# inuyasha2012/vipsy

Hardware: AMD Instinct MI355X
Metric: ELBO-grad steps/sec, 1M persons x 500 items x 100-dim 2PL IRT (higher is better)
Workload: dtype f32

## Files before the change

vipsy_amd/csrc/k_mvn_fwd_b.hip:

```cpp

#define FB_THREADS 256
#define FB_WAVES 4

#define FB_WP 32
#define FB_A_BYTES 8192
#define FB_AUX_BYTES 1024
#define FB_IMG_BYTES (FB_A_BYTES + FB_AUX_BYTES)

__host__ __device__ inline int fb_tiles(int D) { return (pk_off_total(D) + 2 * pk_sec(D)) / 32; }
__host__ __device__ inline int64_t fb_img_floats(int D) {
    return (int64_t)fb_tiles(D) * (FB_IMG_BYTES / 4) + (pk_off_total(D) / 8 + 8 + 3) / 4 * 4;
}
__host__ __device__ inline size_t fb_wave_floats(int D, int J) {
    const size_t w = enc_p_wave_floats(D, J);
    return w < 2048 ? 2048 : w;
}
__host__ __device__ inline size_t fb_lds_bytes(int D, int J) {
    return FB_WAVES * fb_wave_floats(D, J) * sizeof(float) +
           (size_t)(pk_off_total(D) / 8 + 4) / 4 * 16 + 512;
}

#define FB_SC_BLOCKS 64
#define FB_SC_PART 16
#define FB_NSCALES (FB_SC_PART + 4 * FB_SC_BLOCKS)
#define FB_SC_BLOCKS 64
__device__ __forceinline__ void enc_scales_block_max(int blk, int D, int J, const float* __restrict__ W1, const float* __restrict__ b1,
                                                     const float* __restrict__ W21, const float* __restrict__ b21,
                                                     const float* __restrict__ W22, const float* __restrict__ b22,
                                                     float& mw, float& mb, float& m1, float& l1) {
    const int tid = threadIdx.x, lane = tid & 63, wave = tid >> 6;
    const int T = D * (D + 1) / 2;
    const int gt = blk * 256 + tid, gn = FB_SC_BLOCKS * 256;
    mw = 0.f; mb = 0.f; m1 = 0.f; l1 = 0.f;
    auto max4 = [&](const float* __restrict__ w, int n) __attribute__((always_inline)) {
        if (((uintptr_t)w & 15) == 0 && (n & 3) == 0) {
            const f32x4* w4 = (const f32x4*)w;
            const int n4 = n >> 2;
            for (int e = gt; e < n4; e += 4 * gn) {
                f32x4 v[4];
#pragma unroll
                for (int q = 0; q < 4; ++q) v[q] = (e + q * gn < n4) ? w4[e + q * gn] : f32x4{0.f, 0.f, 0.f, 0.f};
#pragma unroll
                for (int q = 0; q < 4; ++q)
                    mw = fmaxf(fmaxf(mw, fmaxf(fabsf(v[q][0]), fabsf(v[q][1]))), fmaxf(fabsf(v[q][2]), fabsf(v[q][3])));
            }
        } else {
            for (int e = gt; e < n; e += gn) mw = fmaxf(mw, fabsf(w[e]));
        }
    };
    max4(W21, D * 64);
    max4(W22, T * 64);
    for (int e = gt; e < D; e += gn) mb = fmaxf(mb, fabsf(b21[e]));
    for (int e = gt; e < T; e += gn) mb = fmaxf(mb, fabsf(b22[e]));
    for (int u = blk * 4 + wave; u < 64; u += FB_SC_BLOCKS * 4) {
        float sacc = 0.f;
        const float* wu = W1 + (int64_t)u * J;
        for (int j0 = 0; j0 < J; j0 += 512) {
            float w[8];
#pragma unroll
            for (int q = 0; q < 8; ++q) w[q] = (j0 + 64 * q + lane < J) ? fabsf(wu[j0 + 64 * q + lane]) : 0.f;
#pragma unroll
            for (int q = 0; q < 8; ++q)
                if (j0 + 64 * q + lane < J) { sacc += w[q]; m1 = fmaxf(m1, w[q]); }
        }
        sacc = wave_sum(sacc) + fabsf(b1[u]);
        l1 = fmaxf(l1, sacc);
    }
    mw = wave_max_dpp(mw); mb = wave_max_dpp(mb); m1 = wave_max_dpp(m1);
}
__global__ __launch_bounds__(256) void k_enc_scales_max(int D, int J, const float* __restrict__ W1, const float* __restrict__ b1,
                                                        const float* __restrict__ W21, const float* __restrict__ b21,
                                                        const float* __restrict__ W22, const float* __restrict__ b22,
                                                        float* __restrict__ sc) {
    float mw, mb, m1, l1;
    enc_scales_block_max(blockIdx.x, D, J, W1, b1, W21, b21, W22, b22, mw, mb, m1, l1);
    if ((threadIdx.x & 63) == 0) {
        uint32_t* w = (uint32_t*)(sc + 11);
        atomicMax(w + 0, __builtin_bit_cast(uint32_t, mw)); atomicMax(w + 1, __builtin_bit_cast(uint32_t, mb));
        atomicMax(w + 2, __builtin_bit_cast(uint32_t, m1)); atomicMax(w + 3, __builtin_bit_cast(uint32_t, l1));
    }
}
__device__ __forceinline__ void enc_scales_from_max(float mw, float mb, float m1, float l1, float* __restrict__ sc) {
    const float hbound = 1.001f * (fmaxf(l1, 0.f) + log1pf(expf(-fabsf(l1)))) + 1e-30f;
    const int sw1 = f16_scale_exp(m1), sh = f16_scale_exp(hbound);
    int sw = f16_scale_exp(mw), sb = f16_scale_exp(mb), eb = sw + sh - sb;
    if (eb > 15) { sw -= eb - 15; eb = 15; }
    if (eb < -14) { sb = sw + sh + 14; eb = -14; }
    sc[0] = ldexpf(1.f, sw1); sc[1] = ldexpf(1.f, -sw1);
    sc[2] = ldexpf(1.f, sw); sc[3] = ldexpf(1.f, sh); sc[4] = ldexpf(1.f, -(sw + sh));
    sc[5] = ldexpf(1.f, sb); sc[6] = ldexpf(1.f, eb);
    sc[7] = hbound; sc[8] = mw; sc[9] = mb; sc[10] = m1;
}
__global__ void k_enc_scales(float* __restrict__ sc) {
    if (threadIdx.x != 0 || blockIdx.x != 0) return;
    enc_scales_from_max(sc[11], sc[12], sc[13], sc[14], sc);
}

template <bool DIRECT = false>
__device__ __forceinline__ void pack_heads_b_tile(int T, int n_off_groups, const float* __restrict__ Wp, const float* __restrict__ bp,
                                                  const uint32_t* __restrict__ gtab, float w_scale, float b_scale,
                                                  uint8_t* __restrict__ img, uint32_t* __restrict__ gt2, int D = 0,
                                                  const float* __restrict__ W21 = nullptr, const float* __restrict__ b21 = nullptr,
                                                  const float* __restrict__ W22 = nullptr, const float* __restrict__ b22 = nullptr,
                                                  uint32_t* __restrict__ gtab_out = nullptr) {
    uint8_t* out = img + (int64_t)T * FB_IMG_BYTES;
    const int tid = threadIdx.x;
    const int Tt = D * (D + 1) / 2;
    if constexpr (DIRECT) {
        if (tid < 4) {
            const int G = 4 * T + tid;
            int src;
            uint32_t c, cn = 0u;
            pk_decode(8 * G, D, Tt, src, c);
            gtab_out[G] = c;
            if (G < n_off_groups) {
                if (G + 1 < n_off_groups) pk_decode(8 * (G + 1), D, Tt, src, cn);
                const uint32_t k = (c >> 12) & 0xFFFFu, l0 = c & 0xFFFu;
                const bool last = (G + 1 == n_off_groups) || (((cn >> 12) & 0xFFFFu) != k);
                gt2[G] = (4u * l0) | ((4u * k) << 12) | (last ? 0x80000000u : 0u);
            }
        }
    } else if (tid < 4 && 4 * T + tid < n_off_groups) {
        const int G = 4 * T + tid;
        const uint32_t c = gtab[G], k = (c >> 12) & 0xFFFFu, l0 = c & 0xFFFu;
        const bool last = (G + 1 == n_off_groups) || (((gtab[G + 1] >> 12) & 0xFFFFu) != k);
        gt2[G] = (4u * l0) | ((4u * k) << 12) | (last ? 0x80000000u : 0u);
    }
    const int row = (tid >> 3) & 31;
    const float* wrow;
    int bsrc = -1;
    if constexpr (DIRECT) {
        uint32_t gc;
        pk_decode(T * 32 + row, D, Tt, bsrc, gc);
        wrow = bsrc < 0 ? nullptr : (bsrc < Tt ? W22 + (int64_t)bsrc * 64 : W21 + (int64_t)(bsrc - Tt) * 64);
    } else {
        wrow = Wp + ((int64_t)T * 32 + row) * 64;
    }
    float v[8];
#pragma unroll
    for (int i = 0; i < 8; ++i) {
        const int e = tid + 256 * i;
        const int j = e & 7, lane = (e >> 3) & 63, sx = e >> 9;
        const int half = lane >> 5;
        v[i] = wrow ? wrow[16 * sx + 8 * (j >> 2) + 4 * half + (j & 3)] : 0.f;
    }
    float bv = 0.f;
    const bool bias_thread = tid < 256 && (tid & 7) < 2;
    if (bias_thread) {
        if constexpr (DIRECT) {
            bv = bsrc < 0 ? 0.f : (bsrc < Tt ? b22[bsrc] : b21[bsrc - Tt]);
        } else {
            bv = bp[T * 32 + (tid >> 3)];
        }
    }
#pragma unroll
    for (int i = 0; i < 8; ++i) {
        const int e = tid + 256 * i;
        const int j = e & 7, lane = (e >> 3) & 63, sx = e >> 9;
        uint16_t* o = (uint16_t*)(out + sx * 1024 + lane * 16) + j;
        split2h_bits(w_scale * v[i], o[0], o[2048]);
    }
    for (int e = tid; e < FB_AUX_BYTES / 2; e += 256) {
        const int j = e & 7;
        uint16_t w = 0;
        if (e < 256 && j < 2) {
            uint16_t bh, bl;
            split2h_bits(b_scale * bv, bh, bl);
            w = j == 0 ? bh : bl;
        }
        ((uint16_t*)(out + FB_A_BYTES))[e] = w;
    }
}
__global__ __launch_bounds__(256) void k_pack_heads_b(int n_tiles, int n_off_groups, const float* __restrict__ Wp, const float* __restrict__ bp,
                               const uint32_t* __restrict__ gtab, const float* __restrict__ sc, uint8_t* __restrict__ img,
                               uint32_t* __restrict__ gt2) {
    if ((int)blockIdx.x >= n_tiles) return;
    pack_heads_b_tile(blockIdx.x, n_off_groups, Wp, bp, gtab, sc[2], sc[5], img, gt2);
}

#define FB_W1_KS 4096
__host__ __device__ inline int64_t fb_w1img_floats(int J) { return (int64_t)((J + 15) / 16) * (FB_W1_KS / 4); }
__device__ __forceinline__ void pack_w1_b_kstep(int ks, int J, const float* __restrict__ W1, float w1_scale, uint8_t* __restrict__ w1img) {
    uint8_t* out = w1img + (int64_t)ks * FB_W1_KS;
    if (blockDim.x != 256) {
        for (int e = threadIdx.x; e < 2 * 64 * 8; e += blockDim.x) {
            const int j = e & 7, lane = (e >> 3) & 63, ht = e >> 9;
            const int half = lane >> 5, hh = 32 * ht + (lane & 31);
            const int it = 16 * ks + 8 * half + j;
            const float w = it < J ? w1_scale * W1[(int64_t)hh * J + it] : 0.f;
            uint16_t* o = (uint16_t*)(out + (ht * 2) * 1024 + lane * 16) + j;
            split2h_bits(w, o[0], o[512]);
        }
        return;
    }
    float v[4];
#pragma unroll
    for (int i = 0; i < 4; ++i) {
        const int e = threadIdx.x + 256 * i;
        const int j = e & 7, lane = (e >> 3) & 63, ht = e >> 9;
        const int half = lane >> 5, hh = 32 * ht + (lane & 31);
        const int it = 16 * ks + 8 * half + j;
        v[i] = it < J ? w1_scale * W1[(int64_t)hh * J + it] : 0.f;
    }
#pragma unroll
    for (int i = 0; i < 4; ++i) {
        const int e = threadIdx.x + 256 * i;
        const int j = e & 7, lane = (e >> 3) & 63, ht = e >> 9;
        uint16_t* o = (uint16_t*)(out + (ht * 2) * 1024 + lane * 16) + j;
        split2h_bits(v[i], o[0], o[512]);
    }
}
__global__ void k_pack_w1_b(int J, const float* __restrict__ W1, const float* __restrict__ sc, uint8_t* __restrict__ w1img) {
    pack_w1_b_kstep(blockIdx.x, J, W1, sc[0], w1img);
}

__device__ __forceinline__ f16x8 fb_y_frag(const uint32_t* yw) {
    typedef uint32_t u32x4y __attribute__((ext_vector_type(4)));
    const uint32_t w0 = yw[0], w1 = yw[1];
    u32x4y q;
#pragma unroll
    for (int d = 0; d < 4; ++d) {
        const uint32_t src = (d >> 1) ? w1 : w0;
        const uint32_t t = (d & 1) ? __builtin_amdgcn_perm(0u, src, 0x0c030c02u) : __builtin_amdgcn_perm(0u, src, 0x0c010c00u);
        q[d] = (t & 0x00010001u) * 0x3C00u | ((t & 0x00800080u) << 8);
    }
    return __builtin_bit_cast(f16x8, q);
}

__device__ __forceinline__ void fb_split8(const float* v, bf16x8& fh, bf16x8& fm, bf16x8& fl) {
    typedef uint32_t u32x4v __attribute__((ext_vector_type(4)));
    u32x4v ph, pm, pl;
#pragma unroll
    for (int q = 0; q < 4; ++q) {
        uint32_t hb[2], mb[2], lb[2];
#pragma unroll
        for (int e = 0; e < 2; ++e) {
            const float x = v[2 * q + e];
            hb[e] = __builtin_bit_cast(uint32_t, x) & 0xffff0000u;
            const float r1 = x - __builtin_bit_cast(float, hb[e]);
            mb[e] = __builtin_bit_cast(uint32_t, r1) & 0xffff0000u;
            const float r2 = r1 - __builtin_bit_cast(float, mb[e]);
            lb[e] = __builtin_bit_cast(uint32_t, r2) & 0xffff0000u;
        }
        ph[q] = hb[1] | (hb[0] >> 16);
        pm[q] = mb[1] | (mb[0] >> 16);
        pl[q] = lb[1] | (lb[0] >> 16);
    }
    fh = __builtin_bit_cast(bf16x8, ph);
    fm = __builtin_bit_cast(bf16x8, pm);
    fl = __builtin_bit_cast(bf16x8, pl);
}

#define FB_SPLIT_MAX 8192
template <bool SPLIT>
__global__ __launch_bounds__(FB_THREADS, 1) void k_mvn_enc_fwd_b(
    EncDims dm, const uint8_t* __restrict__ y, const int64_t* __restrict__ rows, int64_t gid0,
    const uint8_t* __restrict__ w1img, const float* __restrict__ b1, const uint8_t* __restrict__ img,
    const uint32_t* __restrict__ gt2, const float* __restrict__ sc , const float* __restrict__ eps_in, uint64_t seed,
    uint32_t step, const uint32_t* __restrict__ step_dev, uint32_t stream, float* __restrict__ h_out,
    float* __restrict__ x_out, float* __restrict__ eps_out, float* __restrict__ ldT, float* __restrict__ ent_out,
    float* __restrict__ hT_out , float* __restrict__ epsT_out ,
    uint8_t* __restrict__ ximg_out ,
    uint16_t* __restrict__ hs_out ,
    int64_t i_base = 0 ) {
    if (step_dev) step = *step_dev;
    extern __shared__ __attribute__((aligned(16))) float smem[];
    typedef uint32_t u32x4w __attribute__((ext_vector_type(4)));
    constexpr int H = 64;
    const int D = dm.D, J = dm.J;
    const int DS = pk_dse(D), DX = (D + 3) & ~3;
    const int YS = ef_ys(J);
    const int tid = threadIdx.x, lane = tid & 63, wave = __builtin_amdgcn_readfirstlane(tid >> 6);
    const int half = lane >> 5, l31 = lane & 31;
    float* R1 = smem + wave * fb_wave_floats(D, J);
    int8_t* Yi = (int8_t*)R1;
    float* S1 = SPLIT ? smem : R1;
    float* eps_lds = S1;
    float* x_lds = S1 + FB_WP * DS;
    uint32_t* gt_lds = (uint32_t*)(smem + FB_WAVES * fb_wave_floats(D, J));
    float* ent_s = (float*)(gt_lds + ((pk_off_total(D) / 8 + 4) / 4 * 4));
    const int64_t i0 = i_base + (SPLIT ? (int64_t)blockIdx.x * FB_WP : ((int64_t)blockIdx.x * FB_WAVES + wave) * FB_WP);
    const int p = l31;
    const int64_t i = i0 + p;
    const bool wave_live = i0 < dm.nb;
#ifdef FB_STAMPS
    uint64_t fst_[10]; int fsn_ = 0;
#define FSTAMP() do { __builtin_amdgcn_s_waitcnt(0); fst_[fsn_++] = __builtin_amdgcn_s_memtime(); } while (0)
#else
#define FSTAMP() do {} while (0)
#endif
    FSTAMP();

    const int n_off = pk_off_total(D) / 32;
    const int n_sec = pk_sec(D) / 32;
    const int t_end = n_off + 2 * n_sec;
    constexpr int FB_GQ = 5;
    uint32_t gtv[FB_GQ];
#pragma unroll
    for (int q = 0; q < FB_GQ; ++q) { const int e = tid + q * FB_THREADS; gtv[q] = e < 4 * n_off ? gt2[e] : 0u; }
    const float w1_inv = sc[1], h_scale = sc[3], acc_inv = sc[4];

    const int n_ydma = (32 * J + 1023) / 1024;
    const bool ydense = !rows && ((J >> 2) & 1) && i0 + FB_WP <= dm.nb && (i0 * J + (int64_t)n_ydma * 1024 <= dm.nb * (int64_t)J) &&
                        (size_t)n_ydma * 1024 <= fb_wave_floats(D, J) * sizeof(float);
    const int ysr = ydense ? J : YS;
    constexpr int FB_EQ = 16;
    f32x4 zq[FB_EQ];
    const int nblk = D >> 2;
    auto draw_eps = [&]() __attribute__((always_inline)) {
#pragma unroll
        for (int q = 0; q < FB_EQ; ++q) {
            const int e = lane + 64 * q;
            f32x4 z = {0.f, 0.f, 0.f, 0.f};
            if ((!SPLIT || (q & (FB_WAVES - 1)) == wave) && e < FB_WP * nblk) {
                const int pp = e / nblk, blk = e - pp * nblk;
                int64_t ii = i0 + pp;
                if (ii >= dm.nb) ii = dm.nb - 1;
                if (eps_in) {
                    z = *(const f32x4*)(eps_in + ii * D + 4 * blk);
                } else {
                    const int64_t row = rows ? rows[ii] : ii;
                    z = philox_normal4(seed, step, stream, gid0 + row, (uint32_t)blk);
                }
            }
            zq[q] = z;
        }
    };
    if (ydense) {
        const uint8_t* src = y + i0 * J + 16 * lane;
        const uint32_t lb = lds_addr_uniform(R1);
        for (int d = 0; d < n_ydma; ++d) dma16(src + d * 1024, lb + (uint32_t)d * 1024u);
        draw_eps();
        vx_wait_vmem();
    } else {
        constexpr int PB = 16, MAXLD = 4;
        const int YW = YS / 4, JW = J / 4;
        const int nld = (JW + 63) >> 6, nch = (YW + 63) >> 6;
        uint32_t* Yw = (uint32_t*)R1;
        int64_t rowb = 0;
        {
            const int64_t ii = i0 + l31;
            if (ii < dm.nb) rowb = (rows ? rows[ii] : ii) * J;
        }
        const int rowb_lo = (int)(uint32_t)rowb, rowb_hi = (int)(uint32_t)((uint64_t)rowb >> 32);
        if constexpr (SPLIT) {
            const int n_ks_all = (J + 15) / 16, ks_per = (n_ks_all + FB_WAVES - 1) / FB_WAVES;
            const int w_lo = 4 * ks_per * wave;
            const int wpp = 4 * ks_per;
            const int ppl = 64 / wpp > 0 ? 64 / wpp : 1;
            const int pl = lane / wpp, wl = lane - pl * wpp;
            draw_eps();
            for (int p0 = 0; p0 < FB_WP; p0 += ppl * 8) {
                uint32_t v[8];
#pragma unroll
                for (int u = 0; u < 8; ++u) {
                    const int pp = p0 + ppl * u + pl;
                    const int ppc = pp < FB_WP ? pp : FB_WP - 1;
                    const uint64_t rb = ((uint64_t)(uint32_t)__builtin_amdgcn_ds_bpermute(4 * ppc, rowb_hi) << 32) |
                                        (uint32_t)__builtin_amdgcn_ds_bpermute(4 * ppc, rowb_lo);
                    v[u] = 0u;
                    if (pl < ppl && pp < FB_WP && i0 + pp < dm.nb && w_lo + wl < JW) v[u] = ((const uint32_t*)(y + (int64_t)rb))[w_lo + wl];
                }
#pragma unroll
                for (int u = 0; u < 8; ++u) {
                    const int pp = p0 + ppl * u + pl;
                    if (pl < ppl && pp < FB_WP && w_lo + wl < YW) Yw[pp * YW + w_lo + wl] = v[u];
                }
            }
        } else
        for (int p0 = 0; p0 < FB_WP; p0 += PB) {
            uint32_t v[PB][MAXLD];
#pragma unroll
            for (int u = 0; u < PB; ++u) {
                const int pp = p0 + u;
                const uint64_t rb = ((uint64_t)(uint32_t)__builtin_amdgcn_readlane(rowb_hi, pp) << 32) |
                                    (uint32_t)__builtin_amdgcn_readlane(rowb_lo, pp);
                const uint32_t* src = (const uint32_t*)(y + (int64_t)rb) + lane;
                const bool live = i0 + pp < dm.nb;
#pragma unroll
                for (int c = 0; c < MAXLD; ++c) {
                    v[u][c] = 0u;
                    if (c < nld && live && lane + 64 * c < JW) v[u][c] = src[64 * c];
                }
            }
            if (p0 == 0) draw_eps();
#pragma unroll
            for (int u = 0; u < PB; ++u) {
                uint32_t* dst = Yw + (p0 + u) * YW + lane;
#pragma unroll
                for (int c = 0; c < MAXLD + 1; ++c)
                    if (c < nch && lane + 64 * c < YW) dst[64 * c] = c < MAXLD ? v[u][c < MAXLD ? c : 0] : 0u;
            }
        }
    }
#pragma unroll
    for (int q = 0; q < FB_GQ; ++q) { const int e = tid + q * FB_THREADS; if (e < 4 * n_off) gt_lds[e] = gtv[q]; }
    __builtin_amdgcn_wave_barrier();
    FSTAMP();
    f16x8 hb[2][4];
    {
        f32x16 hreg[2];
        f32x16 acc0 = zero16(), acc1 = zero16();
        const int n_ks = (J + 15) / 16;
        auto loadA = [&](f16x8 (&Af)[4], int ks) __attribute__((always_inline)) {
            ks = ks < n_ks ? ks : n_ks - 1;
            const uint8_t* src = w1img + (int64_t)ks * FB_W1_KS + lane * 16;
#pragma unroll
            for (int f = 0; f < 4; ++f) Af[f] = *(const f16x8*)(src + f * 1024);
        };
        auto compute = [&](const f16x8 (&Af)[4], int ks) __attribute__((always_inline)) {
            const f16x8 yb = fb_y_frag((const uint32_t*)(Yi + p * ysr + 16 * ks + 8 * half));
            acc0 = mfma_f16(Af[1], yb, acc0); acc1 = mfma_f16(Af[3], yb, acc1);
            acc0 = mfma_f16(Af[0], yb, acc0); acc1 = mfma_f16(Af[2], yb, acc1);
        };
        if constexpr (SPLIT) {
            const int ks_per = (n_ks + FB_WAVES - 1) / FB_WAVES;
            const int ks_lo = ks_per * wave, ks_hi = (ks_lo + ks_per < n_ks) ? ks_lo + ks_per : n_ks;
            f16x8 A[4][4];
            loadA(A[0], ks_lo); loadA(A[1], ks_lo + 1); loadA(A[2], ks_lo + 2);
            for (int c = ks_lo; c < ks_hi; c += 4) {
#pragma unroll
                for (int u = 0; u < 4; ++u) {
                    loadA(A[(u + 3) & 3], c + u + 3);
                    if (c + u < ks_hi) compute(A[u], c + u);
                }
            }
            __builtin_amdgcn_wave_barrier();
#pragma unroll
            for (int r = 0; r < 16; ++r) { R1[r * 64 + lane] = acc0[r]; R1[(16 + r) * 64 + lane] = acc1[r]; }
            __syncthreads();
            const size_t wstride = fb_wave_floats(D, J);
#pragma unroll
            for (int r = 0; r < 16; ++r) {
                float a0 = smem[r * 64 + lane], a1 = smem[(16 + r) * 64 + lane];
#pragma unroll
                for (int w = 1; w < FB_WAVES; ++w) { a0 += smem[w * wstride + r * 64 + lane]; a1 += smem[w * wstride + (16 + r) * 64 + lane]; }
                acc0[r] = a0; acc1[r] = a1;
            }
            __syncthreads();
        } else {
            f16x8 A[4][4];
            loadA(A[0], 0); loadA(A[1], 1); loadA(A[2], 2);
            for (int c = 0; c < n_ks; c += 4) {
#pragma unroll
                for (int u = 0; u < 4; ++u) {
                    loadA(A[(u + 3) & 3], c + u + 3);
                    if (c + u < n_ks) compute(A[u], c + u);
                }
            }
        }
#pragma unroll
        for (int ht = 0; ht < 2; ++ht) {
#pragma unroll
            for (int g = 0; g < 4; ++g) {
                const int hh0 = 32 * ht + 8 * g + 4 * half;
                const float4 bb = *(const float4*)(b1 + hh0);
                float4 hv;
                hv.x = softplusf_(fmaf((ht ? acc1 : acc0)[4 * g + 0], w1_inv, bb.x));
                hv.y = softplusf_(fmaf((ht ? acc1 : acc0)[4 * g + 1], w1_inv, bb.y));
                hv.z = softplusf_(fmaf((ht ? acc1 : acc0)[4 * g + 2], w1_inv, bb.z));
                hv.w = softplusf_(fmaf((ht ? acc1 : acc0)[4 * g + 3], w1_inv, bb.w));
                hreg[ht][4 * g + 0] = hv.x; hreg[ht][4 * g + 1] = hv.y;
                hreg[ht][4 * g + 2] = hv.z; hreg[ht][4 * g + 3] = hv.w;
                if ((SPLIT ? wave == ht : true) && i < dm.nb) *(float4*)(h_out + i * H + hh0) = hv;
            }
        }
        if (hT_out && i < dm.nb) {
#pragma unroll
            for (int ht = 0; ht < 2; ++ht)
                if (SPLIT ? wave == 2 + ht : true)
#pragma unroll
                    for (int r = 0; r < 16; ++r) hT_out[(int64_t)(32 * ht + crow32(r, half)) * dm.nb + i] = hreg[ht][r];
        }
        if (hs_out && i < dm.nb) {
            const int64_t plane = (int64_t)64 * dm.nb;
#pragma unroll
            for (int ht = 0; ht < 2; ++ht)
                if (SPLIT ? wave == ht : true)
#pragma unroll
                    for (int r = 0; r < 16; ++r) {
                        const int64_t o = (int64_t)(32 * ht + crow32(r, half)) * dm.nb + i;
                        split2h_bits(hreg[ht][r] * h_scale, hs_out[o], hs_out[plane + o]);
                    }
        }
#pragma unroll
        for (int s = 0; s < 4; ++s) {
            float v[8];
#pragma unroll
            for (int j = 0; j < 8; ++j) v[j] = hreg[s >> 1][8 * (s & 1) + j];
            split2h_frag(v, h_scale, hb[0][s], hb[1][s]);
        }
    }
    __builtin_amdgcn_wave_barrier();
    FSTAMP();
    if constexpr (SPLIT) {
        __syncthreads();
        for (int e = tid; e < FB_WP * DX / 4; e += FB_THREADS) *(f32x4*)(x_lds + 4 * e) = f32x4{0.f, 0.f, 0.f, 0.f};
        for (int e = tid; e < FB_WP * (DS - D) / 4; e += FB_THREADS) {
            const int pp = e / ((DS - D) / 4), c = e - pp * ((DS - D) / 4);
            *(f32x4*)(eps_lds + pp * DS + D + 4 * c) = f32x4{0.f, 0.f, 0.f, 0.f};
        }
#pragma unroll
        for (int q = 0; q < FB_EQ; ++q) {
            const int e = lane + 64 * q;
            if ((q & (FB_WAVES - 1)) == wave && e < FB_WP * nblk) {
                const int pp = e / nblk, blk = e - pp * nblk;
                *(f32x4*)(eps_lds + pp * DS + 4 * blk) = zq[q];
                if (i0 + pp < dm.nb) *(f32x4*)(eps_out + (i0 + pp) * D + 4 * blk) = zq[q];
            }
        }
    } else {
        for (int e = lane; e < FB_WP * (DS + DX) / 4; e += 64) *(f32x4*)(S1 + 4 * e) = f32x4{0.f, 0.f, 0.f, 0.f};
        __builtin_amdgcn_wave_barrier();
#pragma unroll
        for (int q = 0; q < FB_EQ; ++q) {
            const int e = lane + 64 * q;
            if (e < FB_WP * nblk) {
                const int pp = e / nblk, blk = e - pp * nblk;
                *(f32x4*)(eps_lds + pp * DS + 4 * blk) = zq[q];
                if (i0 + pp < dm.nb) *(f32x4*)(eps_out + (i0 + pp) * D + 4 * blk) = zq[q];
            }
        }
        __builtin_amdgcn_wave_barrier();
        if (epsT_out && i < dm.nb) {
#pragma unroll 4
            for (int k = half; k < D; k += 2) epsT_out[(int64_t)k * dm.nb + i] = eps_lds[p * DS + k];
        }
    }
    float ent_acc = 0.f;
    const float* ep = eps_lds + p * DS;
    float* xp = x_lds + p * DX;
    struct TileRegs { f16x8 a[2][4]; f16x8 bias; };
    auto pull = [&](TileRegs& R, int t) __attribute__((always_inline)) {
        const int tc = t < t_end ? t : t_end - 1;
        const uint8_t* gb = img + (int64_t)tc * FB_IMG_BYTES + lane * 16;
        R.bias = *(const f16x8*)(gb + FB_A_BYTES);
#pragma unroll
        for (int sp = 1; sp >= 0; --sp)
#pragma unroll
            for (int s = 0; s < 4; ++s) R.a[sp][s] = *(const f16x8*)(gb + (sp * 4 + s) * 1024);
    };
    f16x8 cfrag;
    {
        const _Float16 c16 = (_Float16)sc[6];
#pragma unroll
        for (int j = 0; j < 8; ++j) cfrag[j] = c16;
    }
    auto mma_all = [&](const TileRegs& R) __attribute__((always_inline)) -> f32x16 {
        f32x16 a = mfma_f16(R.bias, cfrag, zero16());
#pragma unroll
        for (int s = 0; s < 4; ++s) a = mfma_f16(R.a[1][s], hb[0][s], a);
#pragma unroll
        for (int s = 0; s < 4; ++s) a = mfma_f16(R.a[0][s], hb[1][s], a);
#pragma unroll
        for (int s = 0; s < 4; ++s) a = mfma_f16(R.a[0][s], hb[0][s], a);
        return a;
    };
    float cur_part = 0.f;
    const char* ep_h = (const char*)(ep + 4 * half);
    char* xp_b = (char*)xp;
    struct EpiOps { float4 e4[4]; };
    auto epi_read = [&](EpiOps& E, const uint4& c) __attribute__((always_inline)) {
        E.e4[0] = *(const float4*)(ep_h + (c.x & 0xFFFu));
        E.e4[1] = *(const float4*)(ep_h + (c.y & 0xFFFu));
        E.e4[2] = *(const float4*)(ep_h + (c.z & 0xFFFu));
        E.e4[3] = *(const float4*)(ep_h + (c.w & 0xFFFu));
    };
    auto epi_group = [&](const f32x16& a, const float4& e, uint32_t code, int g) __attribute__((always_inline)) {
        cur_part = fmaf(a[4 * g + 0], e.x, cur_part);
        cur_part = fmaf(a[4 * g + 1], e.y, cur_part);
        cur_part = fmaf(a[4 * g + 2], e.z, cur_part);
        cur_part = fmaf(a[4 * g + 3], e.w, cur_part);
        if (__builtin_expect((int)code < 0, 0)) {
            const float tot = half_sum32(cur_part) * acc_inv;
            if (half == 0) {
                if (SPLIT) atomicAdd((float*)(xp_b + ((code >> 12) & 0xFFFu)), tot);
                else *(float*)(xp_b + ((code >> 12) & 0xFFFu)) = tot;
            }
            cur_part = 0.f;
        }
    };

    FSTAMP();
    __syncthreads();
    FSTAMP();
    if constexpr (SPLIT) {
        if (epsT_out && i < dm.nb) {
#pragma unroll 4
            for (int k = 2 * wave + half; k < D; k += 2 * FB_WAVES) epsT_out[(int64_t)k * dm.nb + i] = eps_lds[p * DS + k];
        }
    }
    int t_lo = 0, t_hi = n_off;
    if (SPLIT) {
        const int nr = (n_off / 2 < FB_WAVES) ? n_off / 2 : FB_WAVES;
        const int qn = (n_off / nr) & ~1;
        t_lo = wave < nr ? wave * qn : n_off;
        t_hi = (wave >= nr - 1) ? n_off : t_lo + qn;
    }
    TileRegs RA, RB;
    pull(RA, t_lo);
    f32x16 accP = zero16();
    uint4 codeP = make_uint4(0, 0, 0, 0);

    auto off_iter = [&](TileRegs& Rc, TileRegs& Rn, int t, auto firstc) __attribute__((always_inline)) {
        constexpr bool first = decltype(firstc)::value;
        EpiOps E;
        if constexpr (!first) epi_read(E, codeP);
        pull(Rn, t + 1);
        f32x16 a = mfma_f16(Rc.bias, cfrag, zero16());
        a = mfma_f16(Rc.a[1][0], hb[0][0], a);
        a = mfma_f16(Rc.a[1][1], hb[0][1], a);
        if constexpr (!first) epi_group(accP, E.e4[0], codeP.x, 0);
        a = mfma_f16(Rc.a[1][2], hb[0][2], a);
        a = mfma_f16(Rc.a[1][3], hb[0][3], a);
        a = mfma_f16(Rc.a[0][0], hb[1][0], a);
        if constexpr (!first) epi_group(accP, E.e4[1], codeP.y, 1);
        a = mfma_f16(Rc.a[0][1], hb[1][1], a);
        a = mfma_f16(Rc.a[0][2], hb[1][2], a);
        a = mfma_f16(Rc.a[0][3], hb[1][3], a);
        if constexpr (!first) epi_group(accP, E.e4[2], codeP.z, 2);
        a = mfma_f16(Rc.a[0][0], hb[0][0], a);
        a = mfma_f16(Rc.a[0][1], hb[0][1], a);
        if constexpr (!first) epi_group(accP, E.e4[3], codeP.w, 3);
        a = mfma_f16(Rc.a[0][2], hb[0][2], a);
        a = mfma_f16(Rc.a[0][3], hb[0][3], a);
        accP = a;
        const uint4 cv = *(const uint4*)(gt_lds + 4 * t);
        codeP.x = __builtin_amdgcn_readfirstlane(cv.x); codeP.y = __builtin_amdgcn_readfirstlane(cv.y);
        codeP.z = __builtin_amdgcn_readfirstlane(cv.z); codeP.w = __builtin_amdgcn_readfirstlane(cv.w);
    };
    if (!SPLIT || t_lo < t_hi) {
        off_iter(RA, RB, t_lo, std::true_type{});
        off_iter(RB, RA, t_lo + 1, std::false_type{});
        for (int t = t_lo + 2; t < t_hi; t += 2) {
            off_iter(RA, RB, t, std::false_type{});
            off_iter(RB, RA, t + 1, std::false_type{});
        }
        {
            EpiOps E;
            epi_read(E, codeP);
            epi_group(accP, E.e4[0], codeP.x, 0);
            epi_group(accP, E.e4[1], codeP.y, 1);
            epi_group(accP, E.e4[2], codeP.z, 2);
            epi_group(accP, E.e4[3], codeP.w, 3);
        }
        if (SPLIT) {
            const float tot = half_sum32(cur_part) * acc_inv;
            if (half == 0) atomicAdd((float*)(xp_b + ((codeP.w >> 12) & 0xFFFu)), tot);
            cur_part = 0.f;
        }
    }
    FSTAMP();
    if (SPLIT) __syncthreads();
    FSTAMP();
    auto tile_sec = [&](const f32x16& a, int t2) __attribute__((always_inline)) {
        const bool is_diag = t2 < n_off + n_sec;
        const int k0 = 32 * (t2 - (is_diag ? n_off : n_off + n_sec));
#pragma unroll
        for (int g = 0; g < 4; ++g) {
            const int kk = k0 + 8 * g + 4 * half;
            if (kk < D) {
                f32x4 xo = *(const f32x4*)(xp + kk);
                if (is_diag) {
                    const f32x4 ev = *(const f32x4*)(ep + kk);
#pragma unroll
                    for (int j = 0; j < 4; ++j) {
                        const float mkk = a[4 * g + j] * acc_inv;
                        const float ld = __expf(mkk);
                        xo[j] = fmaf(ld, ev[j], xo[j]);
                        ent_acc += mkk;
                        if (i < dm.nb) ldT[(int64_t)(kk + j) * dm.nb + i] = ld;
                    }
                } else {
#pragma unroll
                    for (int j = 0; j < 4; ++j) xo[j] = fmaf(a[4 * g + j], acc_inv, xo[j]);
                }
                *(f32x4*)(xp + kk) = xo;
            }
        }
    };
    auto sec_iter = [&](TileRegs& Rc, TileRegs& Rn, int t) __attribute__((always_inline)) {
        if (t + 1 < t_end) pull(Rn, t + 1);
        const f32x16 a = mma_all(Rc);
        tile_sec(a, t);
    };
    if (SPLIT) {
        for (int ts = wave; ts < n_sec; ts += FB_WAVES) {
            pull(RA, n_off + ts);
            tile_sec(mma_all(RA), n_off + ts);
            pull(RA, n_off + n_sec + ts);
            tile_sec(mma_all(RA), n_off + n_sec + ts);
        }
        const float ea = ent_acc + __shfl_xor(ent_acc, 32, 64);
        if (half == 0) ent_s[wave * FB_WP + p] = ea;
        __syncthreads();
        ent_acc = (ent_s[p] + ent_s[FB_WP + p]) + (ent_s[2 * FB_WP + p] + ent_s[3 * FB_WP + p]);
    } else {
        for (int t = n_off; t < t_end; t += 2) {
            sec_iter(RA, RB, t);
            sec_iter(RB, RA, t + 1);
        }
    }
    vx_wait_vmem();
    __builtin_amdgcn_wave_barrier();
    FSTAMP();
    const int e_lo = SPLIT ? tid : lane, e_st = SPLIT ? FB_THREADS : 64;
    if (ximg_out && i0 < (dm.nb + 63) / 64 * 64) {
        const int pvi = (int)((dm.nb - i0) < FB_WP ? (dm.nb - i0) : FB_WP);
        uint8_t* out = ximg_out + (i0 >> 6) * LH_XT_BYTES;
        const int pbase = (int)(i0 & 63);
        for (int e = e_lo; e < FB_WP * 2 * LB_NKS; e += e_st) {
            int pp, ch;
            if (e < 4 * 3 * 32) {
                const int blk = e >> 5, r = e & 31;
                pp = 8 * (blk / 3) + (r >> 2);
                ch = 4 * (blk % 3) + (r & 3);
            } else {
                const int r = e - 4 * 3 * 32;
                pp = 8 * (r >> 4) + ((r >> 1) & 7);
                ch = 12 + (r & 1);
            }
            float v[8];
#pragma unroll
            for (int j = 0; j < 8; ++j) {
                const int k = 8 * ch + j;
                v[j] = (pp < pvi) ? (k < D ? x_lds[pp * DX + k] : (k == D ? 1.0f : 0.f)) : 0.f;
            }
            f16x8 fh, fl;
            if (lh_split_x(v, fh, fl)) atomicOr((uint32_t*)(ximg_out + (dm.nb + 63) / 64 * (int64_t)LH_XT_BYTES), 1u);
            const uint32_t o = lb_xoff(pbase + pp, ch);
            *(f16x8*)(out + o) = fh;
            *(f16x8*)(out + LB_PLANE + o) = fl;
        }
    }
    if (wave_live) {
        const int pv = (int)((dm.nb - i0) < FB_WP ? (dm.nb - i0) : FB_WP);
        const int c4 = D >> 2;
        for (int e = e_lo; e < pv * c4; e += e_st) {
            const int pp = e / c4, c = e - pp * c4;
            *(f32x4*)(x_out + (i0 + pp) * D + 4 * c) = *(const f32x4*)(x_lds + pp * DX + 4 * c);
        }
        if (!SPLIT) ent_acc += __shfl_xor(ent_acc, 32, 64);
        if ((SPLIT ? wave == FB_WAVES - 1 : true) && half == 0 && i < dm.nb) {
            float s = 0.f;
            for (int k = 0; k < D; k += 4) {
                const f32x4 e = *(const f32x4*)(eps_lds + p * DS + k);
                s += e[0] * e[0]; s += e[1] * e[1]; s += e[2] * e[2]; s += e[3] * e[3];
            }
            ent_out[i] = 0.5f * s + ent_acc;
        }
    }
#ifdef FB_STAMPS
    FSTAMP();
    if (blockIdx.x == 1 && lane == 0)
        printf("FSTAMPS blk %d wave %d: y+draw %llu fc1 %llu eps %llu bar %llu off %llu bar %llu sec %llu out %llu total %llu\n", (int)blockIdx.x, wave,
               fst_[1] - fst_[0], fst_[2] - fst_[1], fst_[3] - fst_[2], fst_[4] - fst_[3], fst_[5] - fst_[4], fst_[6] - fst_[5], fst_[7] - fst_[6],
               fst_[8] - fst_[7], fst_[8] - fst_[0]);
#endif
}


#define NB_THREADS 256
#define NB_WAVES 4
__host__ __device__ inline size_t nb_lds_bytes(int J) {
    return (size_t)NB_WAVES * norm_fast_wave_floats(J) * sizeof(float) + 2 * 6 * 1024;
}

__global__ __launch_bounds__(NB_THREADS, 2) void k_norm_enc_fwd_b(
    EncDims dm, const uint8_t* __restrict__ y, const int64_t* __restrict__ rows, const float* __restrict__ W1,
    const float* __restrict__ b1, const float* __restrict__ W21, const float* __restrict__ b21,
    const float* __restrict__ W22, const float* __restrict__ b22, float* __restrict__ h_out,
    float* __restrict__ loc_out, float* __restrict__ raw_out) {
    extern __shared__ __attribute__((aligned(16))) float smem[];
    typedef uint32_t u32x4w __attribute__((ext_vector_type(4)));
    typedef uint32_t u32x2w __attribute__((ext_vector_type(2)));
    constexpr int H = 64;
    const int J = dm.J, YS = ef_ys(J);
    const int tid = threadIdx.x, lane = tid & 63, wave = tid >> 6, half = lane >> 5, l31 = lane & 31;
    float* R1 = smem + wave * norm_fast_wave_floats(J);
    const int8_t* Yi = (const int8_t*)R1;
    char* frag = (char*)(smem + NB_WAVES * norm_fast_wave_floats(J));
    const int64_t i0 = ((int64_t)blockIdx.x * NB_WAVES + wave) * EP_WP;
    const int p = l31;
    const int64_t i = i0 + p;
    const int n_ydma = (32 * J + 1023) / 1024;
    const bool ydense = !rows && ((J >> 2) & 1) && i0 + EP_WP <= dm.nb && (i0 * J + (int64_t)n_ydma * 1024 <= dm.nb * (int64_t)J);
    const int ysr = ydense ? J : YS;
    if (ydense) {
        const uint8_t* src = y + i0 * J + 16 * lane;
        const uint32_t lb = lds_addr_uniform(R1);
        for (int d = 0; d < n_ydma; ++d) dma16(src + d * 1024, lb + (uint32_t)d * 1024u);
    } else {
        const int YW = YS / 4, JW = J / 4;
        uint32_t* Yw = (uint32_t*)R1;
        const int64_t ip = i0 + l31;
        const int64_t myrow = ip < dm.nb ? (rows ? rows[ip] : ip) : (int64_t)-1;
        const int row_lo = (int)(uint32_t)myrow, row_hi = (int)(uint32_t)((uint64_t)myrow >> 32);
        if (YW >= 64) {
#pragma unroll 4
            for (int pp = 0; pp < EP_WP; ++pp) {
                const int64_t row = (int64_t)(((uint64_t)(uint32_t)__builtin_amdgcn_readlane(row_hi, pp) << 32) |
                                              (uint32_t)__builtin_amdgcn_readlane(row_lo, pp));
                for (int wq = lane; wq < YW; wq += 64) {
                    uint32_t v = 0u;
                    if (wq < JW && row >= 0) v = *(const uint32_t*)(y + row * J + 4 * wq);
                    Yw[pp * YW + wq] = v;
                }
            }
        } else {
#pragma unroll 4
            for (int e = lane; e < EP_WP * YW; e += 64) {
                const int pp = e / YW, wq = e - pp * YW;
                const int64_t row = (int64_t)(((uint64_t)(uint32_t)__shfl(row_hi, pp, 64) << 32) | (uint32_t)__shfl(row_lo, pp, 64));
                uint32_t v = 0u;
                if (wq < JW && row >= 0) v = *(const uint32_t*)(y + row * J + 4 * wq);
                Yw[e] = v;
            }
        }
    }
    const int n_ks = (J + 15) / 16;
    const int hh = tid >> 2, q = tid & 3;
    const float* wrow = W1 + (int64_t)hh * J + 4 * q;
    auto fetch_w = [&](int ks) -> float4 {
        const int j0 = 16 * ks + 4 * q;
        return (ks < n_ks && j0 + 4 <= J) ? *(const float4*)(wrow + 16 * ks) : make_float4(0.f, 0.f, 0.f, 0.f);
    };
    char* wdst = frag + ((hh >> 5) * 3) * 1024 + (32 * (q >> 1) + (hh & 31)) * 16 + 8 * (q & 1);
    auto put_w = [&](const float4& w, int buf) {
        const float v[4] = {w.x, w.y, w.z, w.w};
        uint16_t t[3][4];
#pragma unroll
        for (int e = 0; e < 4; ++e) {
            const __bf16 a = (__bf16)v[e];
            const float r1 = v[e] - (float)a;
            const __bf16 m = (__bf16)r1;
            const __bf16 l = (__bf16)(r1 - (float)m);
            t[0][e] = __builtin_bit_cast(uint16_t, a); t[1][e] = __builtin_bit_cast(uint16_t, m); t[2][e] = __builtin_bit_cast(uint16_t, l);
        }
#pragma unroll
        for (int sp = 0; sp < 3; ++sp) {
            const u32x2w pk = {(uint32_t)t[sp][0] | ((uint32_t)t[sp][1] << 16), (uint32_t)t[sp][2] | ((uint32_t)t[sp][3] << 16)};
            *(u32x2w*)(wdst + buf * 6144 + sp * 1024) = pk;
        }
    };
    put_w(fetch_w(0), 0);
    constexpr int NB_PF = 4;
    float4 wq[NB_PF];
#pragma unroll
    for (int u = 0; u < NB_PF; ++u) wq[u] = fetch_w(1 + u);
    vx_wait_vmem();
    __syncthreads();
    f32x16 acc0 = zero16(), acc1 = zero16();
    for (int ks0 = 0; ks0 < n_ks; ks0 += NB_PF) {
#pragma unroll
      for (int u = 0; u < NB_PF; ++u) {
        const int ks = ks0 + u;
        if (ks >= n_ks) break;
        const int buf = ks & 1;
        const float4 wcur = wq[u];
        wq[u] = fetch_w(ks + 1 + NB_PF);
        const char* fb = frag + buf * 6144 + lane * 16;
        bf16x8 A[6];
#pragma unroll
        for (int f = 0; f < 6; ++f) A[f] = *(const bf16x8*)(fb + f * 1024);
        const uint32_t* yw = (const uint32_t*)(Yi + p * ysr + 16 * ks + 8 * half);
        const u32x2w w = {yw[0], yw[1]};
        u32x4w qv;
#pragma unroll
        for (int d = 0; d < 4; ++d) {
            const uint32_t src = w[d >> 1];
            const uint32_t t = (d & 1) ? __builtin_amdgcn_perm(0u, src, 0x0c030c02u) : __builtin_amdgcn_perm(0u, src, 0x0c010c00u);
            qv[d] = (t & 0x00010001u) * 0x3F80u | ((t & 0x00800080u) << 8);
        }
        const bf16x8 yb = __builtin_bit_cast(bf16x8, qv);
        acc0 = mfma_bf16(A[2], yb, acc0); acc1 = mfma_bf16(A[5], yb, acc1);
        acc0 = mfma_bf16(A[1], yb, acc0); acc1 = mfma_bf16(A[4], yb, acc1);
        acc0 = mfma_bf16(A[0], yb, acc0); acc1 = mfma_bf16(A[3], yb, acc1);
        if (ks + 1 < n_ks) put_w(wcur, buf ^ 1);
        __syncthreads();
      }
    }
    if (i0 >= dm.nb) return;
    float sl = 0.f, sr = 0.f;
#pragma unroll
    for (int ht = 0; ht < 2; ++ht)
#pragma unroll
        for (int g = 0; g < 4; ++g) {
            const int hh0 = 32 * ht + 8 * g + 4 * half;
            const float4 bb = *(const float4*)(b1 + hh0);
            const float4 w21 = make_float4(W21[hh0], W21[hh0 + 1], W21[hh0 + 2], W21[hh0 + 3]);
            const float4 w22 = make_float4(W22[hh0], W22[hh0 + 1], W22[hh0 + 2], W22[hh0 + 3]);
            float4 hv;
            hv.x = softplusf_((ht ? acc1 : acc0)[4 * g + 0] + bb.x);
            hv.y = softplusf_((ht ? acc1 : acc0)[4 * g + 1] + bb.y);
            hv.z = softplusf_((ht ? acc1 : acc0)[4 * g + 2] + bb.z);
            hv.w = softplusf_((ht ? acc1 : acc0)[4 * g + 3] + bb.w);
            sl += hv.x * w21.x + hv.y * w21.y + hv.z * w21.z + hv.w * w21.w;
            sr += hv.x * w22.x + hv.y * w22.y + hv.z * w22.z + hv.w * w22.w;
            if (i < dm.nb) *(float4*)(h_out + i * H + hh0) = hv;
        }
    sl = half_sum32(sl);
    sr = half_sum32(sr);
    if (half == 0 && i < dm.nb) {
        loc_out[i] = sl + b21[0];
        raw_out[i] = sr + b22[0];
    }
}


#define NH_MAX_BLOCKS 64
__host__ __device__ inline int64_t nh_pack_floats(int J) { return fb_w1img_floats(J) + 16 + NH_MAX_BLOCKS; }

__global__ __launch_bounds__(256) void k_norm_pack_max(int J, const float* __restrict__ W1, float* __restrict__ part) {
    __shared__ float red[4];
    float m = 0.f;
    const int n4 = 64 * J / 4;
    const f32x4* w4 = (const f32x4*)W1;
    for (int e = blockIdx.x * 256 + threadIdx.x; e < n4; e += NH_MAX_BLOCKS * 256) {
        const f32x4 v = w4[e];
        m = fmaxf(fmaxf(m, fmaxf(fabsf(v[0]), fabsf(v[1]))), fmaxf(fabsf(v[2]), fabsf(v[3])));
    }
    m = wave_max_dpp(m);
    if ((threadIdx.x & 63) == 0) red[threadIdx.x >> 6] = m;
    __syncthreads();
    if (threadIdx.x == 0) part[blockIdx.x] = fmaxf(fmaxf(red[0], red[1]), fmaxf(red[2], red[3]));
}
__global__ __launch_bounds__(256) void k_norm_pack_w1(int J, const float* __restrict__ W1, const float* __restrict__ part,
                                                      float* __restrict__ sc, uint8_t* __restrict__ w1img) {
    __shared__ float scl;
    if (threadIdx.x < 64) {
        const float m = wave_max_dpp(part[threadIdx.x]);
        if (threadIdx.x == 0) scl = ldexpf(1.f, f16_scale_exp(m));
    }
    __syncthreads();
    if (blockIdx.x == 0 && threadIdx.x == 0) { sc[0] = scl; sc[1] = 1.0f / scl; }
    pack_w1_b_kstep(blockIdx.x, J, W1, scl, w1img);
}

template <int NP>
__host__ __device__ inline size_t nh_wave_floats(int J) {
    const size_t a = (size_t)(32 * NP) * ef_ys(J) / 4, b = (size_t)(((32 * NP * J + 1023) / 1024) * 256);
    return ((a > b ? a : b) + 3) & ~(size_t)3;
}
template <int NP>
__host__ __device__ inline size_t nh_lds_bytes(int J) { return (4 / NP) * nh_wave_floats<NP>(J) * sizeof(float); }

template <int NP, int PF>
__global__ __launch_bounds__(64 * (4 / NP)) void k_norm_enc_fwd_h(
    EncDims dm, const uint8_t* __restrict__ y, const int64_t* __restrict__ rows, const uint8_t* __restrict__ w1img,
    const float* __restrict__ sc, const float* __restrict__ b1, const float* __restrict__ W21, const float* __restrict__ b21,
    const float* __restrict__ W22, const float* __restrict__ b22, float* __restrict__ h_out,
    float* __restrict__ loc_out, float* __restrict__ raw_out) {
    extern __shared__ __attribute__((aligned(16))) float smem[];
    constexpr int H = 64, WP = 32 * NP, NW = 4 / NP, RING = PF + 1;
    const int J = dm.J, YS = ef_ys(J);
    const int tid = threadIdx.x, lane = tid & 63, wave = tid >> 6, half = lane >> 5, l31 = lane & 31;
    float* R1 = smem + wave * nh_wave_floats<NP>(J);
    const int8_t* Yi = (const int8_t*)R1;
    const int64_t i0 = ((int64_t)blockIdx.x * NW + wave) * WP;
    if (i0 >= dm.nb) return;
#ifdef NH_STAMPS
    unsigned long long nst_[5]; int nsn_ = 0;
#define NSTAMP() do { __builtin_amdgcn_s_waitcnt(0); nst_[nsn_++] = __builtin_amdgcn_s_memtime(); } while (0)
#else
#define NSTAMP() do {} while (0)
#endif
    NSTAMP();
    const int n_ydma = (WP * J + 1023) / 1024;
    const bool ydense = !rows && ((J >> 2) & 1) && i0 + WP <= dm.nb && (i0 * J + (int64_t)n_ydma * 1024 <= dm.nb * (int64_t)J);
    const int ysr = ydense ? J : YS;
    const int n_ks = (J + 15) / 16;
    auto loadA = [&](f16x8 (&Af)[4], int ks) __attribute__((always_inline)) {
        ks = ks < n_ks ? ks : n_ks - 1;
        const uint8_t* src = w1img + (int64_t)ks * FB_W1_KS + lane * 16;
#pragma unroll
        for (int f = 0; f < 4; ++f) Af[f] = *(const f16x8*)(src + f * 1024);
    };
    f16x8 A[RING][4];
    if (ydense) {
        const uint8_t* src = y + i0 * J + 16 * lane;
        const uint32_t lb = lds_addr_uniform(R1);
        for (int d = 0; d < n_ydma; ++d) dma16(src + d * 1024, lb + (uint32_t)d * 1024u);
#pragma unroll
        for (int u = 0; u < PF; ++u) loadA(A[u], u);
        vx_wait_vmem();
    } else {
        const int YW = YS / 4, JW = J / 4;
        uint32_t* Yw = (uint32_t*)R1;
        for (int e = lane; e < WP * YW; e += 64) {
            const int pp = e / YW, wq = e - pp * YW;
            const int64_t ii = i0 + pp;
            uint32_t v = 0u;
            if (wq < JW && ii < dm.nb) {
                const int64_t row = rows ? rows[ii] : ii;
// ... 77 lines not shown
```

vipsy_amd/csrc/k_mvn_fwd_b2.hip:

```cpp

#define FB2_THREADS 256
#define FB2_WAVES 4
#define FB2_WP_OF(NS) (32 * (NS))

__host__ __device__ inline size_t fb2_wave_floats(int D, int J, int NS = 2) {
    const size_t a = (size_t)FB2_WP_OF(NS) * ef_ys(J) / 4, b = (size_t)FB2_WP_OF(NS) * pk_dse(D);
    return ((a > b ? a : b) + 3) & ~(size_t)3;
}
__host__ __device__ inline size_t fb2_lds_bytes(int D, int J, int NS = 2) {
    return FB2_WAVES * fb2_wave_floats(D, J, NS) * sizeof(float) + (size_t)(pk_off_total(D) / 8 + 4) / 4 * 16;
}

#define FB2_RING_SLOTS 3
__host__ __device__ inline size_t fb2_tbl_bytes(int D) { return (size_t)(pk_off_total(D) / 8 + 4) / 4 * 16; }
__host__ __device__ inline size_t fb2s_wave_floats(int D) {
    size_t f = (size_t)32 * D + 8;
    if (f < 3072) f = 3072;
    return (f + 3) & ~(size_t)3;
}
__host__ __device__ inline size_t fb2s_lds_bytes(int D) {
    return FB2_WAVES * fb2s_wave_floats(D) * sizeof(float) + fb2_tbl_bytes(D) + (size_t)FB2_RING_SLOTS * FB_IMG_BYTES;
}
__host__ __device__ inline bool fb2s_shape_ok(int D, int J) {
    return D % 4 == 0 && ((D >> 2) & 1) && D >= 80 && J % 4 == 0 && J <= 512 && J > 384 && pk_off_total(D) / 32 >= 4 &&
           2 * ((fb2s_lds_bytes(D) + 1279) / 1280 * 1280) <= 160 * 1024;
}
template <int NS, bool SH = false>
__global__ __launch_bounds__(FB2_THREADS, (NS == 1 ? 2 : 1)) void k_mvn_enc_fwd_b2(
    EncDims dm, const uint8_t* __restrict__ y, const int64_t* __restrict__ rows, int64_t gid0,
    const uint8_t* __restrict__ w1img, const float* __restrict__ b1, const uint8_t* __restrict__ img,
    const uint32_t* __restrict__ gt2, const float* __restrict__ sc , const float* __restrict__ eps_in,
    uint64_t seed, uint32_t step, const uint32_t* __restrict__ step_dev, uint32_t stream, float* __restrict__ h_out, float* __restrict__ x_out, float* __restrict__ eps_out, float* __restrict__ ldT,
    float* __restrict__ ent_out, float* __restrict__ hT_out, float* __restrict__ epsT_out, uint8_t* __restrict__ ximg_out,
    uint16_t* __restrict__ hs_out) {
    if (step_dev) step = *step_dev;
    extern __shared__ __attribute__((aligned(16))) float smem[];
    typedef uint32_t u32x4w __attribute__((ext_vector_type(4)));
    typedef uint32_t u32x2w __attribute__((ext_vector_type(2)));
    constexpr int H = 64, FB2_WP = FB2_WP_OF(NS);
    const int D = dm.D, J = dm.J;
    static_assert(!SH || NS == 1, "shared ring: one person set a wave");
    const int DS = SH ? D : pk_dse(D);
    const int YS = ef_ys(J);
    const int tid = threadIdx.x, lane = tid & 63, wave = __builtin_amdgcn_readfirstlane(tid >> 6);
    const int half = lane >> 5, l31 = lane & 31;
    const size_t WF = SH ? fb2s_wave_floats(D) : fb2_wave_floats(D, J, NS);
    float* R1 = smem + wave * WF;
    int8_t* Yi = (int8_t*)R1;
    float* eps_lds = R1;
    uint32_t* gt_lds = (uint32_t*)(smem + FB2_WAVES * WF);
    uint8_t* ring = (uint8_t*)gt_lds + fb2_tbl_bytes(D);
    const int64_t i0 = ((int64_t)blockIdx.x * FB2_WAVES + wave) * FB2_WP;
    const int p = l31;
    int64_t iu[NS];
#pragma unroll
    for (int u = 0; u < NS; ++u) iu[u] = i0 + 32 * u + p;

#ifdef FB2_STAMPS
    uint64_t st_[10]; int sn_ = 0;
    uint64_t w_lds_ = 0, w_vm_ = 0, w_bar_ = 0;
#define STAMP() do { __builtin_amdgcn_s_waitcnt(0); st_[sn_++] = __builtin_amdgcn_s_memtime(); } while (0)
#else
#define STAMP() do {} while (0)
#endif
    STAMP();
    const int n_off = pk_off_total(D) / 32;
    const int n_sec = pk_sec(D) / 32;
    const int t_end = n_off + 2 * n_sec;
    for (int e = tid; e < 4 * n_off; e += FB2_THREADS) gt_lds[e] = gt2[e];
    const float w1_inv = sc[1], h_scale = sc[3], acc_inv = sc[4];
    const uint32_t ring_lb = SH ? lds_addr_uniform(ring) : 0u;
    auto ring_dma = [&](int t, int slot) __attribute__((always_inline)) {
        const int tc = t < t_end ? t : t_end - 1;
        const uint8_t* gb = img + (int64_t)tc * FB_IMG_BYTES + lane * 16;
        const uint32_t lb = ring_lb + (uint32_t)slot * FB_IMG_BYTES;
        dma16(gb + wave * 1024, lb + (uint32_t)wave * 1024u);
        dma16(gb + (wave + 4) * 1024, lb + (uint32_t)(wave + 4) * 1024u);
        if (wave == 0) dma16(gb + 8 * 1024, lb + 8u * 1024u);
    };
    if constexpr (SH) { ring_dma(0, 0); ring_dma(1, 1); ring_dma(2, 2); }

    const bool qdma = SH && !rows && i0 + FB2_WP <= dm.nb && (i0 + FB2_WP - 1) * (int64_t)J + 512 <= dm.nb * (int64_t)J;
    auto stage_q = [&](int q, int slot) __attribute__((always_inline)) {
        if (qdma) {
            const uint32_t lb = lds_addr_uniform(R1) + (uint32_t)slot * 4096u;
#pragma unroll
            for (int d = 0; d < 4; ++d) {
                const int row = 8 * d + (lane >> 3), pos = lane & 7, c = pos ^ ((row ^ (row >> 3)) & 7);
                dma16(y + (i0 + row) * J + 128 * q + 16 * c, lb + (uint32_t)d * 1024u);
            }
        } else {
            uint32_t* Yw = (uint32_t*)R1 + slot * 1024;
            for (int e = lane; e < 32 * 32; e += 64) {
                const int row = e >> 5, w = e & 31, byte = 128 * q + 4 * w;
                const int64_t ii = i0 + row;
                uint32_t v = 0u;
                if (byte < J && ii < dm.nb) {
                    const int64_t rr = rows ? rows[ii] : ii;
                    v = *(const uint32_t*)(y + rr * J + byte);
                }
                Yw[row * 32 + 4 * ((w >> 2) ^ ((row ^ (row >> 3)) & 7)) + (w & 3)] = v;
            }
        }
    };
    const int n_ydma = (FB2_WP * J + 1023) / 1024;
    const bool ydense = !rows && ((J >> 2) & 1) && i0 + FB2_WP <= dm.nb && (i0 * J + (int64_t)n_ydma * 1024 <= dm.nb * (int64_t)J) &&
                        (size_t)n_ydma * 1024 <= fb2_wave_floats(D, J, NS) * sizeof(float);
    const int ysr = ydense ? J : YS;
    if constexpr (SH) {
        stage_q(0, 0); stage_q(1, 1); stage_q(2, 2);
        if (qdma) vx_wait_vmem();
    } else if (ydense) {
        const uint8_t* src = y + i0 * J + 16 * lane;
        const uint32_t lb = lds_addr_uniform(R1);
        for (int d = 0; d < n_ydma; ++d) dma16(src + d * 1024, lb + (uint32_t)d * 1024u);
        vx_wait_vmem();
    } else {
        const int YW = YS / 4, JW = J / 4;
        uint32_t* Yw = (uint32_t*)R1;
        for (int e = lane; e < FB2_WP * YW; e += 64) {
            const int pp = e / YW, wq = e - pp * YW;
            const int64_t ii = i0 + pp;
            uint32_t v = 0u;
            if (wq < JW && ii < dm.nb) {
                const int64_t row = rows ? rows[ii] : ii;
                v = *(const uint32_t*)(y + row * J + 4 * wq);
            }
            Yw[e] = v;
        }
    }
    __builtin_amdgcn_wave_barrier();
    STAMP();
    f16x8 hb[NS][2][4];
    {
        f32x16 acc[NS][2];
#pragma unroll
        for (int u = 0; u < NS; ++u) { acc[u][0] = zero16(); acc[u][1] = zero16(); }
        const int n_ks = (J + 15) / 16;
        auto loadA = [&](f16x8 (&Af)[4], int ks) __attribute__((always_inline)) {
            ks = ks < n_ks ? ks : n_ks - 1;
            const uint8_t* src = w1img + (int64_t)ks * FB_W1_KS + lane * 16;
#pragma unroll
            for (int f = 0; f < 4; ++f) Af[f] = *(const f16x8*)(src + f * 1024);
        };
        auto compute = [&](const f16x8 (&Af)[4], int ks) __attribute__((always_inline)) {
#pragma unroll
            for (int u = 0; u < NS; ++u) {
                const int8_t* yp = SH ? Yi + ((ks >> 3) == 3 ? 0 : (ks >> 3)) * 4096 + p * 128 + 16 * ((ks & 7) ^ ((p ^ (p >> 3)) & 7)) + 8 * half
                                      : Yi + (32 * u + p) * ysr + 16 * ks + 8 * half;
                const f16x8 yb = fb_y_frag((const uint32_t*)yp);
                acc[u][0] = mfma_f16(Af[1], yb, acc[u][0]); acc[u][1] = mfma_f16(Af[3], yb, acc[u][1]);
                acc[u][0] = mfma_f16(Af[0], yb, acc[u][0]); acc[u][1] = mfma_f16(Af[2], yb, acc[u][1]);
            }
        };
        {
            constexpr int RG = 8;
            f16x8 A[RG][4];
#pragma unroll
            for (int u = 0; u < RG - 1; ++u) loadA(A[u], u);
            for (int c = 0; c < n_ks; c += RG) {
                if constexpr (SH) {
                    if (c == 8) {
                        asm volatile("s_waitcnt lgkmcnt(0)" ::: "memory");
                        __builtin_amdgcn_wave_barrier();
                        stage_q(3, 0);
                    }
                    if (c == 24) {
                        if (qdma) vx_wait_vmem();
                        __builtin_amdgcn_wave_barrier();
                    }
                }
#pragma unroll
                for (int u = 0; u < RG; ++u) {
                    loadA(A[(u + RG - 1) % RG], c + u + RG - 1);
                    if (c + u < n_ks) compute(A[u], c + u);
                }
            }
        }
        STAMP();
        constexpr int ST_T = 36, ST_S = 40;
        constexpr bool SEQ = NS == 1;
        const bool coal = i0 + FB2_WP <= dm.nb && (dm.nb & 7) == 0 && hT_out && hs_out &&
                          (((uintptr_t)hT_out | (uintptr_t)hs_out) & 15) == 0 &&
                          WF * sizeof(float) >= (SEQ ? 128 * ST_S * 2 : 64 * ST_T * 4 + 128 * ST_S * 2);
        float* stT = R1;
        uint16_t* stS = SEQ ? (uint16_t*)R1 : (uint16_t*)(R1 + 64 * ST_T);
#pragma unroll
        for (int u = 0; u < NS; ++u) {
            const int64_t i = iu[u];
            f32x16 hreg[2];
#pragma unroll
            for (int ht = 0; ht < 2; ++ht) {
#pragma unroll
                for (int g = 0; g < 4; ++g) {
                    const int hh0 = 32 * ht + 8 * g + 4 * half;
                    const float4 bb = *(const float4*)(b1 + hh0);
                    float4 hv;
                    hv.x = softplusf_(fmaf(acc[u][ht][4 * g + 0], w1_inv, bb.x));
                    hv.y = softplusf_(fmaf(acc[u][ht][4 * g + 1], w1_inv, bb.y));
                    hv.z = softplusf_(fmaf(acc[u][ht][4 * g + 2], w1_inv, bb.z));
                    hv.w = softplusf_(fmaf(acc[u][ht][4 * g + 3], w1_inv, bb.w));
                    hreg[ht][4 * g + 0] = hv.x; hreg[ht][4 * g + 1] = hv.y;
                    hreg[ht][4 * g + 2] = hv.z; hreg[ht][4 * g + 3] = hv.w;
                    if (i < dm.nb) *(float4*)(h_out + i * H + hh0) = hv;
                }
            }
#pragma unroll
            for (int s = 0; s < 4; ++s) {
                float v[8];
#pragma unroll
                for (int j = 0; j < 8; ++j) v[j] = hreg[s >> 1][8 * (s & 1) + j];
                split2h_frag(v, h_scale, hb[u][0][s], hb[u][1][s]);
            }
            if (coal) {
                __builtin_amdgcn_wave_barrier();
#pragma unroll
                for (int ht = 0; ht < 2; ++ht)
#pragma unroll
                    for (int r = 0; r < 16; ++r) stT[(32 * ht + crow32(r, half)) * ST_T + p] = hreg[ht][r];
                const int64_t c0 = i0 + 32 * u;
                if constexpr (SEQ) {
                    __builtin_amdgcn_wave_barrier();
#ifndef FB2_NO_HT
#pragma unroll
                    for (int it = 0; it < 8; ++it) {
                        const int e = lane + 64 * it, hh = e >> 3, g = e & 7;
                        *(f32x4*)(hT_out + (int64_t)hh * dm.nb + c0 + 4 * g) = *(const f32x4*)(stT + hh * ST_T + 4 * g);
                    }
#endif
                    __builtin_amdgcn_wave_barrier();
                }
#pragma unroll
                for (int t2 = 0; t2 < 2; ++t2)
#pragma unroll
                    for (int s = 0; s < 4; ++s) {
                        const u32x4w w = __builtin_bit_cast(u32x4w, hb[u][t2][s]);
#pragma unroll
                        for (int j = 0; j < 8; ++j) {
                            const int hh = 32 * (s >> 1) + crow32(8 * (s & 1) + j, half);
                            stS[(64 * t2 + hh) * ST_S + p] = (uint16_t)((j & 1) ? (w[j >> 1] >> 16) : (w[j >> 1] & 0xFFFFu));
                        }
                    }
                __builtin_amdgcn_wave_barrier();
                if constexpr (!SEQ) {
#pragma unroll
                    for (int it = 0; it < 8; ++it) {
                        const int e = lane + 64 * it, hh = e >> 3, g = e & 7;
                        *(f32x4*)(hT_out + (int64_t)hh * dm.nb + c0 + 4 * g) = *(const f32x4*)(stT + hh * ST_T + 4 * g);
                    }
                }
#pragma unroll
                for (int it = 0; it < 8; ++it) {
                    const int e = lane + 64 * it, row = e >> 2, g = e & 3;
                    *(u32x4w*)(hs_out + (int64_t)row * dm.nb + c0 + 8 * g) = *(const u32x4w*)(stS + row * ST_S + 8 * g);
                }
            } else if (hT_out && i < dm.nb) {
#pragma unroll
                for (int ht = 0; ht < 2; ++ht)
#pragma unroll
                    for (int r = 0; r < 16; ++r) hT_out[(int64_t)(32 * ht + crow32(r, half)) * dm.nb + i] = hreg[ht][r];
            }
            if (!coal && hs_out && i < dm.nb) {
                const int64_t plane = (int64_t)64 * dm.nb;
#pragma unroll
                for (int ht = 0; ht < 2; ++ht)
#pragma unroll
                    for (int r = 0; r < 16; ++r) {
                        const int64_t o = (int64_t)(32 * ht + crow32(r, half)) * dm.nb + i;
                        split2h_bits(hreg[ht][r] * h_scale, hs_out[o], hs_out[plane + o]);
                    }
            }
        }
    }
    STAMP();
    __builtin_amdgcn_wave_barrier();
    const int nblk = D >> 2;
    for (int e = lane; e < FB2_WP * DS / 4 + (SH ? 2 : 0); e += 64) *(f32x4*)(R1 + 4 * e) = f32x4{0.f, 0.f, 0.f, 0.f};
    __builtin_amdgcn_wave_barrier();
#pragma unroll 5
    for (int e = lane; e < FB2_WP * nblk; e += 64) {
        const int pp = e / nblk, blk = e - pp * nblk;
        int64_t ii = i0 + pp;
        const bool live = ii < dm.nb;
        if (!live) ii = dm.nb - 1;
        f32x4 z;
        if (eps_in) {
            z = *(const f32x4*)(eps_in + ii * D + 4 * blk);
        } else {
            const int64_t row = rows ? rows[ii] : ii;
            z = philox_normal4(seed, step, stream, gid0 + row, (uint32_t)blk);
        }
        *(f32x4*)(eps_lds + pp * DS + 4 * blk) = z;
    }
    __builtin_amdgcn_wave_barrier();
    const bool coalE = i0 + FB2_WP <= dm.nb && (dm.nb & 3) == 0 && epsT_out && ((uintptr_t)epsT_out & 15) == 0;
    if (coalE) {
        constexpr int PG = FB2_WP / 4;
        for (int e = lane; e < D * PG; e += 64) {
            const int k = e / PG, g = e - k * PG;
            const float* ec = eps_lds + 4 * g * DS + k;
            *(f32x4*)(epsT_out + (int64_t)k * dm.nb + i0 + 4 * g) = f32x4{ec[0], ec[DS], ec[2 * DS], ec[3 * DS]};
        }
    }
    float eps2[NS];
#pragma unroll
    for (int u = 0; u < NS; ++u) {
        const float* er = eps_lds + (32 * u + p) * DS;
        if (!coalE && epsT_out && iu[u] < dm.nb) {
#pragma unroll 4
            for (int k = half; k < D; k += 2) epsT_out[(int64_t)k * dm.nb + iu[u]] = er[k];
        }
        float s2 = 0.f;
        for (int k = 0; k < D; ++k) s2 = fmaf(er[k], er[k], s2);
        eps2[u] = s2;
    }
    STAMP();
    struct TileRegs { f16x8 a[2][4]; f16x8 bias; };
    auto pull = [&](TileRegs& R, int t) __attribute__((always_inline)) {
        const int tc = t < t_end ? t : t_end - 1;
        const uint8_t* gb = img + (int64_t)tc * FB_IMG_BYTES + lane * 16;
        R.bias = *(const f16x8*)(gb + FB_A_BYTES);
#pragma unroll
        for (int sp = 1; sp >= 0; --sp)
#pragma unroll
            for (int s = 0; s < 4; ++s) R.a[sp][s] = *(const f16x8*)(gb + (sp * 4 + s) * 1024);
    };
    f16x8 cfrag;
    {
        const _Float16 c16 = (_Float16)sc[6];
#pragma unroll
        for (int j = 0; j < 8; ++j) cfrag[j] = c16;
    }
    auto mma_all = [&](const TileRegs& R, int u) __attribute__((always_inline)) -> f32x16 {
        f32x16 a = mfma_f16(R.bias, cfrag, zero16());
#pragma unroll
        for (int s = 0; s < 4; ++s) a = mfma_f16(R.a[1][s], hb[u][0][s], a);
#pragma unroll
        for (int s = 0; s < 4; ++s) a = mfma_f16(R.a[0][s], hb[u][1][s], a);
#pragma unroll
        for (int s = 0; s < 4; ++s) a = mfma_f16(R.a[0][s], hb[u][0][s], a);
        return a;
    };
    float cur_part[NS];
    const char* ep_h[NS];
    float* xrow[NS];
    float* xst[NS];
    const bool whole = i0 + FB2_WP <= dm.nb;
    const int st_sh = whole ? (NS == 2 ? 6 : 5) : 0;
#pragma unroll
    for (int u = 0; u < NS; ++u) {
        cur_part[u] = 0.f;
        ep_h[u] = (const char*)(eps_lds + (32 * u + p) * DS + 4 * half);
        xrow[u] = x_out + (iu[u] < dm.nb ? iu[u] : dm.nb - 1) * D;
        xst[u] = whole ? eps_out + i0 * D + 32 * u + p : xrow[u];
    }
    struct EpiOps { float4 e4[NS][4]; };
    auto epi_read = [&](EpiOps& E, const uint4& c) __attribute__((always_inline)) {
#pragma unroll
        for (int u = 0; u < NS; ++u) {
            E.e4[u][0] = *(const float4*)(ep_h[u] + (c.x & 0xFFFu));
            E.e4[u][1] = *(const float4*)(ep_h[u] + (c.y & 0xFFFu));
            E.e4[u][2] = *(const float4*)(ep_h[u] + (c.z & 0xFFFu));
            E.e4[u][3] = *(const float4*)(ep_h[u] + (c.w & 0xFFFu));
        }
    };
    auto epi_group = [&](const f32x16 (&a)[NS], const EpiOps& E, uint32_t code, int g) __attribute__((always_inline)) {
#pragma unroll
        for (int j = 0; j < 4; ++j)
#pragma unroll
            for (int u = 0; u < NS; ++u) {
                const float ev = j == 0 ? E.e4[u][g].x : j == 1 ? E.e4[u][g].y : j == 2 ? E.e4[u][g].z : E.e4[u][g].w;
                float av = a[u][4 * g + j];
                if (g == 0 && j == 0) av = __builtin_bit_cast(float, __builtin_amdgcn_mov_dpp(__builtin_bit_cast(int, av), 0xE4, 0xF, 0xF, true));
                asm volatile("v_fmac_f32 %0, %1, %2" : "+v"(cur_part[u]) : "v"(av), "v"(ev));
            }
        if (__builtin_expect((int)code < 0, 0)) {
#pragma unroll
            for (int u = 0; u < NS; ++u) {
                const float tot = half_sum32(cur_part[u]) * acc_inv;
                if (half == 0 && iu[u] < dm.nb) *(float*)((char*)xst[u] + (((code >> 12) & 0xFFFu) << st_sh)) = tot;
                cur_part[u] = 0.f;
            }
        }
    };

    if constexpr (SH) vx_wait_vmem();
    __syncthreads();
    TileRegs RA, RB;
    int s_rd = 1;
    auto ring_read = [&](TileRegs& R, int slot) __attribute__((always_inline)) {
        const uint8_t* lb = ring + slot * FB_IMG_BYTES + lane * 16;
        R.bias = *(const f16x8*)(lb + FB_A_BYTES);
#pragma unroll
        for (int sp = 1; sp >= 0; --sp)
#pragma unroll
            for (int s = 0; s < 4; ++s) R.a[sp][s] = *(const f16x8*)(lb + (sp * 4 + s) * 1024);
    };
    f32x16 accP[NS];
#pragma unroll
    for (int u = 0; u < NS; ++u) accP[u] = zero16();
    uint4 codeP = make_uint4(0, 0, 0, 0);
    auto off_iter = [&](TileRegs& Rc, TileRegs& Rn, int t, auto firstc) __attribute__((always_inline)) {
        constexpr bool first = decltype(firstc)::value;
        EpiOps E;
        if constexpr (!first) epi_read(E, codeP);
        if constexpr (SH) ring_read(Rn, s_rd); else pull(Rn, t + 1);
        f32x16 a[NS];
#pragma unroll
        for (int u = 0; u < NS; ++u) a[u] = mfma_f16(Rc.bias, cfrag, zero16());
#pragma unroll
        for (int s = 0; s < 2; ++s)
#pragma unroll
            for (int u = 0; u < NS; ++u) a[u] = mfma_f16(Rc.a[1][s], hb[u][0][s], a[u]);
        if constexpr (!first) epi_group(accP, E, codeP.x, 0);
#pragma unroll
        for (int s = 2; s < 4; ++s)
#pragma unroll
            for (int u = 0; u < NS; ++u) a[u] = mfma_f16(Rc.a[1][s], hb[u][0][s], a[u]);
#pragma unroll
        for (int u = 0; u < NS; ++u) a[u] = mfma_f16(Rc.a[0][0], hb[u][1][0], a[u]);
        if constexpr (!first) epi_group(accP, E, codeP.y, 1);
#pragma unroll
        for (int s = 1; s < 4; ++s)
#pragma unroll
            for (int u = 0; u < NS; ++u) a[u] = mfma_f16(Rc.a[0][s], hb[u][1][s], a[u]);
        if constexpr (!first) epi_group(accP, E, codeP.z, 2);
#pragma unroll
        for (int s = 0; s < 2; ++s)
#pragma unroll
            for (int u = 0; u < NS; ++u) a[u] = mfma_f16(Rc.a[0][s], hb[u][0][s], a[u]);
        if constexpr (!first) epi_group(accP, E, codeP.w, 3);
#pragma unroll
        for (int s = 2; s < 4; ++s)
#pragma unroll
            for (int u = 0; u < NS; ++u) a[u] = mfma_f16(Rc.a[0][s], hb[u][0][s], a[u]);
#pragma unroll
        for (int u = 0; u < NS; ++u) accP[u] = a[u];
        const uint4 cv = *(const uint4*)(gt_lds + 4 * t);
        codeP.x = __builtin_amdgcn_readfirstlane(cv.x); codeP.y = __builtin_amdgcn_readfirstlane(cv.y);
        codeP.z = __builtin_amdgcn_readfirstlane(cv.z); codeP.w = __builtin_amdgcn_readfirstlane(cv.w);
        if constexpr (SH) {
#ifdef FB2_STAMPS
            const uint64_t tw0_ = __builtin_amdgcn_s_memtime();
#endif
            asm volatile("s_waitcnt lgkmcnt(0)" ::: "memory");
#ifdef FB2_STAMPS
            const uint64_t tw1_ = __builtin_amdgcn_s_memtime();
#endif
            if (wave == 0) __builtin_amdgcn_s_waitcnt(0x0F70 | 3); else __builtin_amdgcn_s_waitcnt(0x0F70 | 2);
#ifdef FB2_STAMPS
            const uint64_t tw2_ = __builtin_amdgcn_s_memtime();
#endif
            __builtin_amdgcn_s_barrier();
#ifdef FB2_STAMPS
            { const uint64_t tw3_ = __builtin_amdgcn_s_memtime(); w_lds_ += tw1_ - tw0_; w_vm_ += tw2_ - tw1_; w_bar_ += tw3_ - tw2_; }
#endif
            ring_dma(t + 4, s_rd);
            s_rd = s_rd == FB2_RING_SLOTS - 1 ? 0 : s_rd + 1;
        }
    };
    if constexpr (SH) {
        ring_read(RA, 0);
        asm volatile("s_waitcnt lgkmcnt(0)" ::: "memory");
        __builtin_amdgcn_s_barrier();
        ring_dma(3, 0);
    } else {
        pull(RA, 0);
    }
    off_iter(RA, RB, 0, std::true_type{});
    off_iter(RB, RA, 1, std::false_type{});
    for (int t = 2; t < n_off; t += 2) {
        off_iter(RA, RB, t, std::false_type{});
        off_iter(RB, RA, t + 1, std::false_type{});
    }
    {
        EpiOps E;
        epi_read(E, codeP);
        epi_group(accP, E, codeP.x, 0);
        epi_group(accP, E, codeP.y, 1);
        epi_group(accP, E, codeP.z, 2);
        epi_group(accP, E, codeP.w, 3);
    }
    vx_wait_vmem();
    STAMP();
    float ent_acc[NS];
#pragma unroll
    for (int u = 0; u < NS; ++u) ent_acc[u] = 0.f;
    pull(RA, n_off);
    pull(RB, n_off + n_sec);
    for (int kb = 0; kb < n_sec; ++kb) {
        const int k0 = 32 * kb;
        if (k0 >= D) break;
        f32x4 xo[NS][4];
#pragma unroll
        for (int u = 0; u < NS; ++u) {
#pragma unroll
            for (int g = 0; g < 4; ++g) {
                const int kk = k0 + 8 * g + 4 * half;
#pragma unroll
                for (int j = 0; j < 4; ++j) xo[u][g][j] = (kk < D) ? xst[u][(int64_t)(kk + j) << st_sh] : 0.f;
            }
            if (k0 == 0 && half == 0) xo[u][0][0] = 0.f;
        }
        f32x16 aD[NS], aL[NS];
#pragma unroll
        for (int u = 0; u < NS; ++u) aD[u] = mma_all(RA, u);
        pull(RA, n_off + kb + 1);
#pragma unroll
        for (int u = 0; u < NS; ++u) aL[u] = mma_all(RB, u);
        pull(RB, n_off + n_sec + kb + 1);
#pragma unroll
        for (int u = 0; u < NS; ++u) {
            const bool live = iu[u] < dm.nb;
            const float* er = eps_lds + (32 * u + p) * DS;
#pragma unroll
            for (int g = 0; g < 4; ++g) {
                const int kk = k0 + 8 * g + 4 * half;
                if (kk < D) {
                    const f32x4 ev = *(const f32x4*)(er + kk);
                    f32x4 xn;
#pragma unroll
                    for (int j = 0; j < 4; ++j) {
                        const float mkk = aD[u][4 * g + j] * acc_inv;
                        const float ld = __expf(mkk);
                        xn[j] = fmaf(aL[u][4 * g + j], acc_inv, fmaf(ld, ev[j], xo[u][g][j]));
                        ent_acc[u] += mkk;
                        if (live) ldT[(int64_t)(kk + j) * dm.nb + iu[u]] = ld;
                    }
                    if (live) *(f32x4*)(xrow[u] + kk) = xn;
                }
            }
        }
    }
    vx_wait_vmem();
    for (int e = lane; e < FB2_WP * nblk; e += 64) {
        const int pp = e / nblk, blk = e - pp * nblk;
        if (i0 + pp < dm.nb) *(f32x4*)(eps_out + (i0 + pp) * D + 4 * blk) = *(const f32x4*)(eps_lds + pp * DS + 4 * blk);
    }
#pragma unroll
    for (int u = 0; u < NS; ++u) {
        ent_acc[u] += __shfl_xor(ent_acc[u], 32, 64);
        if (half == 0 && iu[u] < dm.nb) ent_out[iu[u]] = 0.5f * eps2[u] + ent_acc[u];
    }
    STAMP();
    if (ximg_out && i0 < (dm.nb + 63) / 64 * 64) {
        const int pbase = (int)(i0 & 63);
        vx_wait_vmem();
        __builtin_amdgcn_wave_barrier();
        const int pvi = (int)((dm.nb - i0) < FB2_WP ? (dm.nb - i0) : FB2_WP);
        uint8_t* out = ximg_out + (i0 >> 6) * LH_XT_BYTES;
        constexpr int XU = 7;
        static_assert((FB2_WP * 2 * LB_NKS) % (64 * XU) == 0, "x image work items");
        for (int e0 = lane; e0 < FB2_WP * 2 * LB_NKS; e0 += 64 * XU) {
            f32x4 q[XU][2];
            uint32_t off[XU];
#pragma unroll
            for (int w = 0; w < XU; ++w) {
                const int e = e0 + 64 * w;
                const int hs2 = e / (32 * 2 * LB_NKS), e2 = e - hs2 * (32 * 2 * LB_NKS);
                int pp, ch;
                if (e2 < 4 * 3 * 32) {
                    const int blk = e2 >> 5, r = e2 & 31;
                    pp = 8 * (blk / 3) + (r >> 2);
                    ch = 4 * (blk % 3) + (r & 3);
                } else {
                    const int r = e2 - 4 * 3 * 32;
                    pp = 8 * (r >> 4) + ((r >> 1) & 7);
                    ch = 12 + (r & 1);
                }
                pp += 32 * hs2;
                off[w] = lb_xoff(pbase + pp, ch);
                const float* xr = x_out + (i0 + (pp < pvi ? pp : 0)) * D;
#pragma unroll
                for (int h2 = 0; h2 < 2; ++h2) {
                    const int k0 = 8 * ch + 4 * h2;
                    f32x4 v = {0.f, 0.f, 0.f, 0.f};
                    if (pp < pvi) {
                        if (k0 < D) v = *(const f32x4*)(xr + k0);
                        else if (k0 == D) v[0] = 1.0f;
                    }
                    q[w][h2] = v;
                }
            }
#pragma unroll
            for (int w = 0; w < XU; ++w) {
                float v[8];
#pragma unroll
                for (int j = 0; j < 8; ++j) v[j] = q[w][j >> 2][j & 3];
                f16x8 fh, fl;
                if (lh_split_x(v, fh, fl)) atomicOr((uint32_t*)(ximg_out + (dm.nb + 63) / 64 * (int64_t)LH_XT_BYTES), 1u);
                *(f16x8*)(out + off[w]) = fh;
                *(f16x8*)(out + LB_PLANE + off[w]) = fl;
            }
        }
    }
#ifdef FB2_STAMPS
    STAMP();
    if ((blockIdx.x == 100 || blockIdx.x == 2000 || blockIdx.x == 5000) && lane == 0 && (wave == 0 || wave == 3))
        printf("STAMPS blk %d wave %d: y %llu fc1 %llu hout %llu eps %llu off %llu sec %llu ximg %llu total %llu | turn waits: lds %llu dma %llu barrier %llu\n",
               (int)blockIdx.x, wave, st_[1] - st_[0], st_[2] - st_[1], st_[3] - st_[2], st_[4] - st_[3], st_[5] - st_[4], st_[6] - st_[5],
               st_[7] - st_[6], st_[7] - st_[0], w_lds_, w_vm_, w_bar_);
#endif
}
```

vipsy_amd/csrc/k_mvn_score_b.hip:

```cpp
#pragma once

#define SB_THREADS 256
#define SB_WAVES 4
#define SB_WP 32

__host__ __device__ inline int sb_col_jb0(int c) { return c & ~3; }
__host__ __device__ inline int sb_col_tiles(int D, int c) { return (D - sb_col_jb0(c) + 31) / 32; }
__host__ __device__ inline int sb_tiles(int D) {
    int n = 0;
    for (int c = 0; c < D; ++c) n += sb_col_tiles(D, c);
    return n;
}
__host__ __device__ inline int sb_ds(int D) {
    int ds = (D + 32 + 3) & ~3;
    if (((ds >> 2) & 1) == 0) ds += 4;
    return ds;
}
__host__ __device__ inline size_t sb_lds_bytes(int D) { return (size_t)SB_WAVES * SB_WP * sb_ds(D) * sizeof(float); }
#define SBR_CONSUMERS 8
#define SBR_THREADS (64 * (SBR_CONSUMERS + 1))
__host__ __device__ inline size_t sbr_lds_bytes(int D) {
    return (size_t)SBR_CONSUMERS * SB_WP * sb_ds(D) * sizeof(float) + 2 * (size_t)FB_IMG_BYTES;
}
__host__ __device__ inline int64_t sb_img_floats(int D) { return (int64_t)sb_tiles(D) * (FB_IMG_BYTES / 4); }

__global__ __launch_bounds__(256) void k_pack_heads_col(int D, const float* __restrict__ W22, const float* __restrict__ b22,
                                                       const float* __restrict__ sc, uint8_t* __restrict__ img) {
    int t = blockIdx.x, c = D - 1;
    while (c > 0 && t >= sb_col_tiles(D, c)) { t -= sb_col_tiles(D, c); --c; }
    const int jb = sb_col_jb0(c) + 32 * t;
    const float w_scale = sc[2], b_scale = sc[5];
    uint8_t* out = img + (int64_t)blockIdx.x * FB_IMG_BYTES;
    const int tid = threadIdx.x;
    const int row = (tid >> 3) & 31;
    const int j = jb + row;
    const bool live = j >= c && j < D;
    const int64_t src = (int64_t)j * (j + 1) / 2 + c;
    const float* wrow = W22 + src * 64;
    float v[8];
#pragma unroll
    for (int i = 0; i < 8; ++i) {
        const int e = tid + 256 * i;
        const int jj = e & 7, lane = (e >> 3) & 63, sx = e >> 9;
        const int half = lane >> 5;
        v[i] = live ? wrow[16 * sx + 8 * (jj >> 2) + 4 * half + (jj & 3)] : 0.f;
    }
    const float bv = (live && (tid & 7) < 2) ? b22[src] : 0.f;
#pragma unroll
    for (int i = 0; i < 8; ++i) {
        const int e = tid + 256 * i;
        const int jj = e & 7, lane = (e >> 3) & 63, sx = e >> 9;
        uint16_t* o = (uint16_t*)(out + sx * 1024 + lane * 16) + jj;
        split2h_bits(w_scale * v[i], o[0], o[2048]);
    }
    for (int e = tid; e < FB_AUX_BYTES / 2; e += 256) {
        const int jj = e & 7;
        uint16_t w = 0;
        if (e < 256 && jj < 2) {
            uint16_t bh, bl;
            split2h_bits(b_scale * bv, bh, bl);
            w = jj == 0 ? bh : bl;
        }
        ((uint16_t*)(out + FB_A_BYTES))[e] = w;
    }
}

template <bool RING>
__global__ __launch_bounds__(RING ? SBR_THREADS : SB_THREADS, RING ? 1 : 2) void k_mvn_score_b(
    int D, int64_t nb, float scale, const int64_t* __restrict__ rows, const float* __restrict__ h ,
    const uint8_t* __restrict__ img, const float* __restrict__ sc, const float* __restrict__ eps ,
    const float* __restrict__ ll, const float* __restrict__ ent, float* __restrict__ baseline, float base_beta, int base_by_row,
    float* __restrict__ log_r_out, float* __restrict__ gxT , float* __restrict__ gdT ) {
    extern __shared__ __attribute__((aligned(16))) float sb_lds[];
    const int DS = sb_ds(D);
    const int tid = threadIdx.x, lane = tid & 63, wave = __builtin_amdgcn_readfirstlane(tid >> 6);
    const int half = lane >> 5, p = lane & 31;
    constexpr int NCW = RING ? SBR_CONSUMERS : SB_WAVES;
    const int n_tiles = sb_tiles(D);
    typedef __attribute__((address_space(3))) uint8_t lds_u8;
    lds_u8* const ring = (lds_u8*)(sb_lds + (size_t)NCW * SB_WP * DS);
    auto turn = [&]() __attribute__((always_inline)) {
        asm volatile("" ::: "memory");
        __builtin_amdgcn_s_waitcnt(0xC07F);
        __builtin_amdgcn_s_barrier();
        asm volatile("" ::: "memory");
    };
    if constexpr (RING) {
        if (wave == NCW) {
            const uint32_t ring_l = lds_addr_uniform((const void*)(sb_lds + (size_t)NCW * SB_WP * DS));
            auto stage = [&](int t) __attribute__((always_inline)) {
                const int tc = t < n_tiles ? t : n_tiles - 1;
                const uint8_t* gb = img + (int64_t)tc * FB_IMG_BYTES + lane * 16;
                const uint32_t dst = ring_l + (uint32_t)(t & 1) * FB_IMG_BYTES;
#pragma unroll
                for (int f = 0; f < 9; ++f) dma16(gb + f * 1024, __builtin_amdgcn_readfirstlane(dst + (uint32_t)f * 1024u));
            };
            stage(0); stage(1);
            vx_wait_vmem();
            turn();
            turn();
            for (int t = 0; t < n_tiles; ++t) {
                stage(t + 2);
                vx_wait_vmem();
                turn();
            }
            return;
        }
    }
    float* const u_t = sb_lds + (size_t)wave * SB_WP * DS;
    const int64_t i0 = ((int64_t)blockIdx.x * NCW + wave) * SB_WP;
    if constexpr (!RING)
        if (i0 >= nb) return;
    const int64_t i = i0 + p;
    const bool live = i < nb;
    const int64_t ic = live ? i : nb - 1;
    const float h_scale = sc[3], acc_inv = sc[4];

    float w;
    {
        const float lr = scale * (ll[ic] + ent[ic]);
        w = lr;
        if (baseline) {
            const int64_t bi = (base_by_row && rows) ? rows[ic] : ic;
            const float bv = baseline[bi];
            w = lr - bv;
            if (live && half == 0 && base_beta >= 0.f) baseline[bi] = fmaf(base_beta, bv, (1.0f - base_beta) * lr);
        }
        if (live && half == 0 && log_r_out) log_r_out[i] = lr;
    }
    f16x8 hb[2][4];
    {
        const float* hr = h + ic * 64 + 4 * half;
        f32x4 q[8];
#pragma unroll
        for (int s = 0; s < 4; ++s) { q[2 * s] = *(const f32x4*)(hr + 16 * s); q[2 * s + 1] = *(const f32x4*)(hr + 16 * s + 8); }
#pragma unroll
        for (int s = 0; s < 4; ++s) {
            const float v[8] = {q[2 * s][0], q[2 * s][1], q[2 * s][2], q[2 * s][3], q[2 * s + 1][0], q[2 * s + 1][1], q[2 * s + 1][2], q[2 * s + 1][3]};
            split2h_frag(v, h_scale, hb[0][s], hb[1][s]);
        }
    }
    {
        const int c4 = D >> 2, z4 = (DS - D) >> 2;
        for (int e = lane; e < SB_WP * c4; e += 64) {
            const int pp = e / c4, cq = e - pp * c4;
            int64_t ii = i0 + pp;
            ii = ii < nb ? ii : nb - 1;
            *(f32x4*)(u_t + pp * DS + 4 * cq) = *(const f32x4*)(eps + ii * D + 4 * cq);
        }
        for (int e = lane; e < SB_WP * z4; e += 64) {
            const int pp = e / z4, cq = e - pp * z4;
            *(f32x4*)(u_t + pp * DS + D + 4 * cq) = f32x4{0.f, 0.f, 0.f, 0.f};
        }
    }
    __builtin_amdgcn_wave_barrier();
    __builtin_amdgcn_s_waitcnt(0xC07F);
    float* const up = u_t + p * DS;

    struct TileRegs { f16x8 a[2][4]; f16x8 bias; };
    auto pull = [&](TileRegs& R, int t) __attribute__((always_inline)) {
        if constexpr (RING) {
            lds_u8* lb = ring + (t & 1) * FB_IMG_BYTES + lane * 16;
            R.bias = *(const __attribute__((address_space(3))) f16x8*)(lb + FB_A_BYTES);
#pragma unroll
            for (int sp = 1; sp >= 0; --sp)
#pragma unroll
                for (int s = 0; s < 4; ++s) R.a[sp][s] = *(const __attribute__((address_space(3))) f16x8*)(lb + (sp * 4 + s) * 1024);
        } else {
            const int tc = t < n_tiles ? t : n_tiles - 1;
            const uint8_t* gb = img + (int64_t)tc * FB_IMG_BYTES + lane * 16;
            R.bias = *(const f16x8*)(gb + FB_A_BYTES);
#pragma unroll
            for (int sp = 1; sp >= 0; --sp)
#pragma unroll
                for (int s = 0; s < 4; ++s) R.a[sp][s] = *(const f16x8*)(gb + (sp * 4 + s) * 1024);
        }
    };
    f16x8 cfrag;
    {
        const _Float16 c16 = (_Float16)sc[6];
#pragma unroll
        for (int j = 0; j < 8; ++j) cfrag[j] = c16;
    }
    int c = D - 1, jb = sb_col_jb0(c), left = sb_col_tiles(D, c);
    bool fst = true;
    int cP = 0, jbP = 0;
    bool endP = false, fstP = false;
    float dot = 0.f, lcc = 1.f, rlc = 1.f, e_c = 0.f;
    f32x16 accP = zero16();
    const float* up_h = up + 4 * half;
    f32x4 uq[4];
    auto epi_read = [&]() __attribute__((always_inline)) {
#pragma unroll
        for (int g = 0; g < 4; ++g) uq[g] = *(const f32x4*)(up_h + jbP + 8 * g);
    };
    auto epi_group = [&](int g) __attribute__((always_inline)) {
        dot = fmaf(accP[4 * g + 0], uq[g][0], dot);
        dot = fmaf(accP[4 * g + 1], uq[g][1], dot);
        dot = fmaf(accP[4 * g + 2], uq[g][2], dot);
        dot = fmaf(accP[4 * g + 3], uq[g][3], dot);
    };
    auto column_start = [&]() __attribute__((always_inline)) {
        const int q = cP & 3;
        const float m = q == 0 ? accP[0] : (q == 1 ? accP[1] : (q == 2 ? accP[2] : accP[3]));
        e_c = up[cP];
        if (half == 0) {
            dot = fmaf(-m, e_c, dot);
            lcc = __expf(m * acc_inv);
            rlc = fast_rcp(lcc);
        }
    };
    auto column_end = [&]() __attribute__((always_inline)) {
        const float tot = half_sum32(dot) * acc_inv;
        if (half == 0) {
            const float uc = (e_c - tot) * rlc;
            up[cP] = uc;
            if (live) {
                const float g = w * uc;
                gxT[(int64_t)cP * nb + i] = g;
                if (gdT) gdT[(int64_t)cP * nb + i] = fmaf(g * e_c, lcc, -w);
            }
        }
        dot = 0.f;
    };
    auto tile_iter = [&](TileRegs& Rc, TileRegs& Rn, int t, auto firstc) __attribute__((always_inline)) {
        constexpr bool first = decltype(firstc)::value;
        if constexpr (!first) epi_read();
        pull(Rn, t + 1);
        f32x16 a = mfma_f16(Rc.bias, cfrag, zero16());
        a = mfma_f16(Rc.a[1][0], hb[0][0], a);
        a = mfma_f16(Rc.a[1][1], hb[0][1], a);
        if constexpr (!first) epi_group(0);
        a = mfma_f16(Rc.a[1][2], hb[0][2], a);
        a = mfma_f16(Rc.a[1][3], hb[0][3], a);
        a = mfma_f16(Rc.a[0][0], hb[1][0], a);
        if constexpr (!first) epi_group(1);
        a = mfma_f16(Rc.a[0][1], hb[1][1], a);
        a = mfma_f16(Rc.a[0][2], hb[1][2], a);
        a = mfma_f16(Rc.a[0][3], hb[1][3], a);
        if constexpr (!first) epi_group(2);
        a = mfma_f16(Rc.a[0][0], hb[0][0], a);
        a = mfma_f16(Rc.a[0][1], hb[0][1], a);
        if constexpr (!first) epi_group(3);
        a = mfma_f16(Rc.a[0][2], hb[0][2], a);
        a = mfma_f16(Rc.a[0][3], hb[0][3], a);
        if constexpr (!first) {
            if (fstP) column_start();
            if (endP) column_end();
        }
        accP = a;
        cP = c; jbP = jb; endP = (left == 1); fstP = fst;
        if (left == 1) {
            --c;
            jb = sb_col_jb0(c);
            left = c >= 0 ? sb_col_tiles(D, c) : 1;
            fst = true;
        } else {
            jb += 32;
            --left;
            fst = false;
        }
        if constexpr (RING) turn();
    };
    TileRegs RA, RB;
    if constexpr (RING) {
        turn();
        pull(RA, 0);
        turn();
    } else {
        pull(RA, 0);
    }
    tile_iter(RA, RB, 0, std::true_type{});
    int t = 1;
    for (; t + 1 < n_tiles; t += 2) {
        tile_iter(RB, RA, t, std::false_type{});
        tile_iter(RA, RB, t + 1, std::false_type{});
    }
    if (t < n_tiles) tile_iter(RB, RA, t, std::false_type{});
    epi_read();
    epi_group(0); epi_group(1); epi_group(2); epi_group(3);
    if (fstP) column_start();
    column_end();
}
```

vipsy_amd/csrc/k_pack_fused.hip:

```cpp
#pragma once

__device__ __forceinline__ void rows_from_ring(const int64_t* __restrict__ ring, int64_t ring_stride, int ring_slots,
                                               const uint32_t* __restrict__ step_dev, int64_t* __restrict__ rows_out, int64_t nb) {
    const int64_t* src = ring + (int64_t)(*step_dev % (uint32_t)ring_slots) * ring_stride;
    for (int64_t i = threadIdx.x; i < nb; i += blockDim.x) rows_out[i] = __builtin_nontemporal_load(src + i);
}
__global__ __launch_bounds__(256) void k_rows_from_ring(const int64_t* __restrict__ ring, int64_t ring_stride, int ring_slots,
                                                        const uint32_t* __restrict__ step_dev, int64_t* __restrict__ rows_out,
                                                        int64_t nb) {
    rows_from_ring(ring, ring_stride, ring_slots, step_dev, rows_out, nb);
}

__global__ __launch_bounds__(256) void k_pack_stage1(int D, int J, const float* __restrict__ W1, const float* __restrict__ b1,
                                                     const float* __restrict__ W21, const float* __restrict__ b21,
                                                     const float* __restrict__ W22, const float* __restrict__ b22,
                                                     float* __restrict__ Wp, float* __restrict__ bp, uint32_t* __restrict__ gtab,
                                                     float* __restrict__ WpT ,
                                                     float* __restrict__ sc, const int64_t* __restrict__ ring = nullptr,
                                                     int64_t ring_stride = 0, int ring_slots = 1,
                                                     const uint32_t* __restrict__ step_dev = nullptr,
                                                     int64_t* __restrict__ rows_out = nullptr, int64_t nb = 0,
                                                     int n_row_blocks = -1 ) {
    if (n_row_blocks < 0) n_row_blocks = (pk_rows(D) + 3) / 4;
    const int Rp = pk_rows(D);
    const int blk = blockIdx.x, tid = threadIdx.x;
    if (blk == n_row_blocks + FB_SC_BLOCKS) {
        rows_from_ring(ring, ring_stride, ring_slots, step_dev, rows_out, nb);
        return;
    }
    if (blk < n_row_blocks) {
        const int T = D * (D + 1) / 2;
        const int pr = 4 * blk + (tid >> 6), hh = tid & 63;
        if (pr >= Rp) return;
        int src;
        uint32_t gcode;
        pk_decode(pr, D, T, src, gcode);
        const float v = (src < 0) ? 0.f : (src < T ? W22[(int64_t)src * 64 + hh] : W21[(int64_t)(src - T) * 64 + hh]);
        Wp[(int64_t)pr * 64 + hh] = v;
        if (WpT) WpT[(int64_t)hh * Rp + pr] = v;
        if (hh == 0) {
            bp[pr] = (src < 0) ? 0.f : (src < T ? b22[src] : b21[src - T]);
            if ((pr & 7) == 0) gtab[pr >> 3] = gcode;
        }
        return;
    }
    const int b = blk - n_row_blocks;
    __shared__ float red[4][4];
    float mw, mb, m1, l1;
    enc_scales_block_max(b, D, J, W1, b1, W21, b21, W22, b22, mw, mb, m1, l1);
    if ((tid & 63) == 0) { red[tid >> 6][0] = mw; red[tid >> 6][1] = mb; red[tid >> 6][2] = m1; red[tid >> 6][3] = l1; }
    __syncthreads();
    if (tid < 4) sc[FB_SC_PART + 4 * b + tid] = fmaxf(fmaxf(red[0][tid], red[1][tid]), fmaxf(red[2][tid], red[3][tid]));
}

__global__ __launch_bounds__(256) void k_pack_stage2(int D, int J, int n_tiles, int n_off_groups, const float* __restrict__ W1,
                                                     const float* __restrict__ W21, const float* __restrict__ W22,
                                                     const float* __restrict__ Wp, const float* __restrict__ bp,
                                                     const uint32_t* __restrict__ gtab, float* __restrict__ sc,
                                                     uint8_t* __restrict__ w1img, uint8_t* __restrict__ img, uint32_t* __restrict__ gt2,
                                                     uint8_t* __restrict__ himg ,
                                                     const float* __restrict__ b21 = nullptr ,
                                                     const float* __restrict__ b22 = nullptr, uint32_t* __restrict__ gtab_out = nullptr) {
    __shared__ float scl[16];
    const int tid = threadIdx.x, blk = blockIdx.x;
    if (tid < 64) {
        const f32x4 v = *(const f32x4*)(sc + FB_SC_PART + 4 * tid);
        const float mw = wave_max_dpp(v[0]), mb = wave_max_dpp(v[1]), m1 = wave_max_dpp(v[2]), l1 = wave_max_dpp(v[3]);
        if (tid == 0) enc_scales_from_max(mw, mb, m1, l1, scl);
    }
    __syncthreads();
    if (blk == 0) {
        if (tid < 11) sc[tid] = scl[tid];
        else if (tid < 15) ((uint32_t*)sc)[tid] = 0u;
    }
    const int n_w1 = (J + 15) / 16;
    if (blk < n_w1) { pack_w1_b_kstep(blk, J, W1, scl[0], w1img); return; }
    if (blk < n_w1 + n_tiles) {
        if (gtab_out) pack_heads_b_tile<true>(blk - n_w1, n_off_groups, Wp, bp, gtab, scl[2], scl[5], img, gt2, D, W21, b21, W22, b22, gtab_out);
        else pack_heads_b_tile<false>(blk - n_w1, n_off_groups, Wp, bp, gtab, scl[2], scl[5], img, gt2);
        return;
    }
    if (himg) pack_heads_hb_unit(blk - n_w1 - n_tiles, D, W21, W22, scl[2], himg);
}

__global__ __launch_bounds__(256) void k_enc_bwd_tail(int D, int H, const float* __restrict__ slabs_w, int n_prw, int64_t lenw,
                                                      float alpha, float* __restrict__ out_w, int n_unpack,
                                                      const float* __restrict__ slabs_f, int64_t n_prf, int64_t lenf,
                                                      float* __restrict__ out_f, int n_f1, const float* __restrict__ ll,
                                                      const float* __restrict__ ent, int64_t nb, float loss_alpha,
                                                      float* __restrict__ loss, float* __restrict__ sum_ws,
                                                      uint32_t* __restrict__ tick) {
    __shared__ float part[4][64];
    const int blk = blockIdx.x;
    if (blk < n_unpack) { unpack_head_rows(blk, D, H, slabs_w, n_prw, lenw, alpha, out_w); return; }
    if (blk < n_unpack + n_f1) { reduce_slabs_cols(blk - n_unpack, n_f1, part, slabs_f, n_prf, lenf, lenf, alpha, out_f); return; }
    if (ll) sum_block(0, 1, &part[0][0], ll, nb, sum_ws, ent, loss_alpha, loss, tick);
}

__global__ __launch_bounds__(BT_THREADS, 1) void k_bwd_wt_fc1(
    EncDims dm, const float* __restrict__ hT, const float* __restrict__ epsT, const float* __restrict__ gdT,
    const float* __restrict__ gxT, const uint32_t* __restrict__ gtab, float* __restrict__ slabs_w, int64_t lenw, int wt_gx, int wt_gy,
    const uint8_t* __restrict__ y, const int64_t* __restrict__ rows, const float* __restrict__ ghpre, float* __restrict__ slabs_f,
    int64_t lenf, int fast, int f_gx, int f_gy) {
    extern __shared__ __attribute__((aligned(16))) char smem_wf[];
    const int L = blockIdx.x, n_wt = wt_gx * wt_gy;
    if (L < n_wt) {
        bwd_w_t_body(dm, hT, epsT, gdT, gxT, gtab, slabs_w, lenw, smem_wf, VGrid{L, wt_gx, wt_gy});
        return;
    }
    const int Lf = L - n_wt;
    fc1_bwd_body<2, 1>(dm, y, rows, ghpre, slabs_f, lenf, fast, (float*)smem_wf, Lf % f_gx, Lf / f_gx, f_gy);
}
```

vipsy_amd/csrc/vx_abi.hip:

```cpp
#include "vx_common.h"
#include "k_util.hip"
#include "k_mvn_enc.hip"
#include "k_mvn_enc_fast.hip"
#include "k_mvn_enc_r.hip"
#include "k_mvn_packed.hip"
#include "k_mvn_enc_bwd.hip"
#include "k_mvn_enc_bwd_fast.hip"
#include "k_irt_lik.hip"
#include "k_irt_lik_r.hip"
#include "k_irt_lik_b.hip"
#include "k_irt_lik_h.hip"
#include "k_irt1d.hip"
#include "k_irt1d_sparse.hip"
#include "k_hodina.hip"
#include "k_hodina_m.hip"
#include "k_norm_enc.hip"
#include "k_mvn_bbvi.hip"
#include "k_mvn_score.hip"
#include "k_mvn_bwd_t.hip"
#include "k_mvn_bwd_b.hip"
#include "k_mvn_fwd_b.hip"
#include "k_mvn_fwd_b2.hip"
#include "k_mvn_score_b.hip"
#include "k_mvn_bwd_hb.hip"
#include "k_mvn_bwd_hb2.hip"
#include "k_pack_fused.hip"
#include "k_fc1_bwd_c.hip"
#include "k_cdm_sf.hip"
#include "k_synth.hip"
#include "k_vaeccdm.hip"

#include <unordered_map>
#include <mutex>
#include <cstdlib>
#include <cstring>
#include <vector>
#include <utility>
#include <optional>
#include <cstdio>

namespace {

int g_num_cu = 0;
int num_cu() {
    if (g_num_cu == 0) {
        int dev = 0;
        hipDeviceProp_t prop;
        if (hipGetDevice(&dev) == hipSuccess && hipGetDeviceProperties(&prop, dev) == hipSuccess)
            g_num_cu = prop.multiProcessorCount;
        if (g_num_cu <= 0) g_num_cu = 256;
    }
    return g_num_cu;
}

inline int set_lds_ptr(const void* kernel, size_t bytes) {
    if (bytes > 160 * 1024) return VX_EINVAL;
    static std::mutex mu;
    static std::unordered_map<const void*, size_t> have;
    std::lock_guard<std::mutex> lock(mu);
    auto it = have.find(kernel);
    if (it != have.end() && it->second >= bytes) return VX_OK;
    hipError_t e = hipFuncSetAttribute(kernel, hipFuncAttributeMaxDynamicSharedMemorySize, (int)bytes);
    if (e != hipSuccess) return (int)e;
    have[kernel] = bytes;
    return VX_OK;
}
template <typename K>
int set_lds(K kernel, size_t bytes) { return set_lds_ptr(reinterpret_cast<const void*>(kernel), bytes); }

inline int grid_1d(int64_t n, int block) {
    int64_t g = (n + block - 1) / block;
    const int64_t cap = (int64_t)num_cu() * 8;
    return (int)(g < 1 ? 1 : (g > cap ? cap : g));
}

inline int tril_len(int D) { return D * (D + 1) / 2; }

EncDims make_enc_dims(const vx_irt_cfg* cfg, int64_t nb) {
    EncDims dm;
    dm.D = cfg->D; dm.J = cfg->J; dm.H = cfg->H;
    dm.Hp = (cfg->H + 31) / 32 * 32;
    dm.DS = enc_ds(cfg->D);
    dm.T = tril_len(cfg->D);
    dm.nb = nb;
    return dm;
}

inline bool aligned16(const void* p) { return (reinterpret_cast<uintptr_t>(p) & 15u) == 0; }

struct Seams {
    bool generic;
    bool fwd16, w16, h16, fc1_16;
    bool side_streams;
    bool fwd_ring, score_ring;
};
const Seams& seams() {
    static const Seams s = [] {
        Seams v;
        const char *g = getenv("VX_FORCE_GENERIC"), *m = getenv("VX_MFMA16"), *r = getenv("VX_FWD_RING");
        v.generic = g && g[0] == '1';
        const int mode = (!m || m[0] == '1') ? 15 : (m[0] == 'f' ? 1 : m[0] == 'w' ? 2 : m[0] == 'h' ? 4 : m[0] == 'g' ? 8 : 0);
        v.fwd16 = mode & 1; v.w16 = mode & 2; v.h16 = mode & 4; v.fc1_16 = mode & 8;
        v.side_streams = v.fc1_16;
        v.fwd_ring = !(r && r[0] == '0');
        v.score_ring = getenv("VX_SCORE_NO_RING") == nullptr;
        return v;
    }();
    return s;
}
bool force_generic() { return seams().generic; }

bool packed_ok(const vx_irt_cfg* cfg) {
    return !force_generic() && cfg->H == 64 && cfg->J % 4 == 0 && cfg->D % 4 == 0 &&
           enc_p_lds_floats(cfg->D, cfg->J) * sizeof(float) <= 160 * 1024 &&
           enc_bwdw_fast_lds_floats(cfg->D) * sizeof(float) <= 160 * 1024;
}
bool fwb_shape(const vx_irt_cfg* cfg) {
    return seams().fwd16 && packed_ok(cfg) && cfg->D <= 128 && fb_lds_bytes(cfg->D, cfg->J) <= 160 * 1024;
}

bool enc_cfg_ok(const vx_irt_cfg* cfg) {
    return cfg && cfg->D >= 2 && cfg->D <= 127 && cfg->H >= 1 && cfg->H <= 128 && cfg->J >= 1;
}


struct ProfSlot { const char* name; int64_t units; std::vector<std::pair<hipEvent_t, hipEvent_t>> ev; };
bool g_prof = false;
ProfSlot g_prof_slots[12];
int g_prof_n = 0;
struct ProfScope {
    hipEvent_t a = nullptr, b = nullptr;
    hipStream_t st;
    const char* name;
    int64_t units;
    ProfScope(const char* nm, hipStream_t s, int64_t u = 0, bool on = true) : st(s), name(nm), units(u) {
        if (!g_prof || !on) return;
        if (hipEventCreate(&a) != hipSuccess || hipEventCreate(&b) != hipSuccess) { a = nullptr; return; }
        (void)hipEventRecord(a, st);
    }
    void cancel() {
        if (a) { (void)hipEventDestroy(a); a = nullptr; }
        if (b) { (void)hipEventDestroy(b); b = nullptr; }
    }
    ~ProfScope() {
        if (!a) return;
        (void)hipEventRecord(b, st);
        for (int i = 0; i < g_prof_n; ++i)
            if (!strcmp(g_prof_slots[i].name, name)) { g_prof_slots[i].units = units; g_prof_slots[i].ev.emplace_back(a, b); return; }
        if (g_prof_n < 12) {
            g_prof_slots[g_prof_n].name = name; g_prof_slots[g_prof_n].units = units;
            g_prof_slots[g_prof_n].ev.emplace_back(a, b); ++g_prof_n; return;
        }
        (void)hipEventDestroy(a); (void)hipEventDestroy(b);
    }
};

struct SideStream {
    hipStream_t s = nullptr;
    hipEvent_t fork = nullptr, join = nullptr;
    bool init = false, ok = false;
};
SideStream& side_stream(int which, hipStream_t main_st) {
    constexpr int MAXDEV = 16, MAXMAIN = 4;
    struct Slot { hipStream_t main_st = nullptr; SideStream ss[2]; bool used = false; uint64_t last = 0; };
    struct Slots {
        Slot s[MAXDEV][MAXMAIN];
        uint64_t clock = 0;
        static void release(Slot& sl) {
            for (SideStream& x : sl.ss) {
                if (x.s) (void)hipStreamDestroy(x.s);
                if (x.fork) (void)hipEventDestroy(x.fork);
                if (x.join) (void)hipEventDestroy(x.join);
                x = SideStream();
            }
            sl.used = false;
        }
        ~Slots() {
            for (auto& d : s) for (Slot& sl : d) if (sl.used) release(sl);
        }
    };
    static thread_local Slots slots;
    static thread_local SideStream none;
    int dev = -1;
    if (hipGetDevice(&dev) != hipSuccess || dev < 0 || dev >= MAXDEV) return none;
    Slot* sl = nullptr;
    for (int i = 0; i < MAXMAIN && !sl; ++i)
        if (slots.s[dev][i].used && slots.s[dev][i].main_st == main_st) sl = &slots.s[dev][i];
    for (int i = 0; i < MAXMAIN && !sl; ++i)
        if (!slots.s[dev][i].used) { sl = &slots.s[dev][i]; sl->used = true; sl->main_st = main_st; }
    if (!sl) {
        sl = &slots.s[dev][0];
        for (int i = 1; i < MAXMAIN; ++i)
            if (slots.s[dev][i].last < sl->last) sl = &slots.s[dev][i];
        Slots::release(*sl);
        sl->used = true;
        sl->main_st = main_st;
    }
    sl->last = ++slots.clock;
    SideStream& ss = sl->ss[which & 1];
    if (!ss.init) {
        ss.init = true;
        ss.ok = hipStreamCreateWithFlags(&ss.s, hipStreamNonBlocking) == hipSuccess &&
                hipEventCreateWithFlags(&ss.fork, hipEventDisableTiming) == hipSuccess &&
                hipEventCreateWithFlags(&ss.join, hipEventDisableTiming) == hipSuccess;
    }
    return ss;
}
struct ForkScope {
    SideStream* ss = nullptr;
    hipStream_t main_st = nullptr;
    bool fork(SideStream& s, hipStream_t st) {
        if (!s.ok || hipEventRecord(s.fork, st) != hipSuccess || hipStreamWaitEvent(s.s, s.fork, 0) != hipSuccess) return false;
        ss = &s; main_st = st;
        return true;
    }
    bool active() const { return ss != nullptr; }
    hipStream_t side() const { return ss->s; }
    int join() {
        if (!ss) return VX_OK;
        SideStream* s = ss;
        ss = nullptr;
        if (hipEventRecord(s->join, s->s) != hipSuccess || hipStreamWaitEvent(main_st, s->join, 0) != hipSuccess) return VX_EINVAL;
        return VX_OK;
    }
    ~ForkScope() { (void)join(); }
};

}

extern "C" {

int vx_abi_version(void) { return VX_ABI_VERSION; }
const char* vx_build_info(void) { return "vipsy_amd gfx950 fp32-mfma " __DATE__ " " __TIME__; }

int vx_prof_enable(int on) {
    if (on == 2 || on == 3) { g_prof = on == 2; return VX_OK; }
    for (int i = 0; i < g_prof_n; ++i) {
        for (auto& e : g_prof_slots[i].ev) { (void)hipEventDestroy(e.first); (void)hipEventDestroy(e.second); }
        g_prof_slots[i].ev.clear();
    }
    g_prof_n = 0;
    g_prof = on != 0;
    return VX_OK;
}

int vx_prof_count(void) { return g_prof_n; }

int vx_prof_read(int slot, char* name, int name_cap, float* mean_ms, int* launches) {
    if (slot < 0 || slot >= g_prof_n || !name || name_cap < 1 || !mean_ms || !launches) return VX_EINVAL;
    const ProfSlot& s = g_prof_slots[slot];
    strncpy(name, s.name, (size_t)name_cap - 1);
    name[name_cap - 1] = 0;
    double tot = 0;
    for (auto& e : s.ev) {
        float ms = 0.f;
        if (hipEventSynchronize(e.second) != hipSuccess || hipEventElapsedTime(&ms, e.first, e.second) != hipSuccess)
            return VX_EINVAL;
        tot += ms;
    }
    *launches = (int)s.ev.size();
    *mean_ms = s.ev.empty() ? 0.f : (float)(tot / s.ev.size());
    return VX_OK;
}

int vx_prof_units(int slot, int64_t* units) {
    if (slot < 0 || slot >= g_prof_n || !units) return VX_EINVAL;
    *units = g_prof_slots[slot].units;
    return VX_OK;
}

int vx_philox_normals(float* eps, const int64_t* gids, int64_t gid0, int64_t n, int32_t D, uint64_t seed,
                      uint32_t step, uint32_t stream, void* hs) {
    if (!eps || n < 0 || D < 1) return VX_EINVAL;
    if (n == 0) return VX_OK;
    const int64_t total = n * ((D + 3) / 4);
    hipLaunchKernelGGL(k_philox_normals, dim3(grid_1d(total, 256)), dim3(256), 0, (hipStream_t)hs, eps, gids,
                       gid0, n, (int)D, seed, step, stream);
    VX_CHECK_LAUNCH();
    return VX_OK;
}

int vx_philox_raw(uint32_t* out, int64_t gid0, int64_t n, uint64_t seed, uint32_t step, uint32_t stream,
                  void* hs) {
    if (!out || n < 0) return VX_EINVAL;
    if (n == 0) return VX_OK;
    hipLaunchKernelGGL(k_philox_raw, dim3(grid_1d(n, 256)), dim3(256), 0, (hipStream_t)hs, out, gid0, n, seed,
                       step, stream);
    VX_CHECK_LAUNCH();
    return VX_OK;
}

int vx_reduce_slabs(const float* slabs, int64_t n_slabs, int64_t len, float alpha, float* out, void* hs) {
    if (!slabs || !out || n_slabs < 1 || len < 0) return VX_EINVAL;
    if (len == 0) return VX_OK;
    if (n_slabs <= 8 && len >= (1 << 16) && len % 4 == 0 && aligned16(slabs) && aligned16(out)) {
        hipLaunchKernelGGL(k_reduce_few, dim3(num_cu() * 8), dim3(256), 0, (hipStream_t)hs, (const float4*)slabs,
                           (int)n_slabs, len / 4, len / 4, alpha, (float4*)out);
        VX_CHECK_LAUNCH();
        return VX_OK;
    }
    hipLaunchKernelGGL(k_reduce_slabs, dim3(grid_1d(len, 64)), dim3(256), 0, (hipStream_t)hs, slabs, n_slabs,
                       len, len, alpha, out);
    VX_CHECK_LAUNCH();
    return VX_OK;
}

static int reduce_step_slabs(const float* slabs, int64_t n_slabs, int J, float* gitem, float* loss, uint32_t* tick,
                             void* hs, const vx_adam_tail* opt = nullptr) {
    const int64_t len = 4 * (int64_t)J + (loss ? 1 : 0);
    if (opt) {
        if (!loss || !opt->pA || !opt->mA || !opt->vA || !opt->segsA || opt->nA != 4 * (int64_t)J || opt->n_segsA < 1 ||
            opt->n_segsA > VX_MAX_SEGS || opt->nB < 0 || opt->n_segsB < 0 || opt->n_segsB > VX_MAX_SEGS ||
            (opt->nB > 0 && (!opt->pB || !opt->gB || !opt->mB || !opt->vB || !opt->segsB || opt->n_segsB < 1)) ||
            (opt->t < 1 && !tick))
            return VX_EINVAL;
        AdamSegs sa, sb;
        sa.n = opt->n_segsA; sb.n = opt->nB > 0 ? opt->n_segsB : 0;
        for (int i = 0; i < sa.n; ++i) {
            if (opt->segsA[i].begin < 0 || opt->segsA[i].end > opt->nA || opt->segsA[i].begin > opt->segsA[i].end) return VX_EINVAL;
            sa.begin[i] = opt->segsA[i].begin; sa.end[i] = opt->segsA[i].end; sa.lr[i] = opt->segsA[i].lr;
        }
        for (int i = 0; i < sb.n; ++i) {
            if (opt->segsB[i].begin < 0 || opt->segsB[i].end > opt->nB || opt->segsB[i].begin > opt->segsB[i].end) return VX_EINVAL;
            sb.begin[i] = opt->segsB[i].begin; sb.end[i] = opt->segsB[i].end; sb.lr[i] = opt->segsB[i].lr;
        }
        const AdamBuf A{opt->pA, gitem, opt->mA, opt->vA, opt->freeA, opt->nA}, B{opt->pB, opt->gB, opt->mB, opt->vB, nullptr, opt->nB};
        const double bc1 = 1.0 - pow((double)opt->beta1, (double)(tick ? 1 : opt->t));
        const double bc2 = 1.0 - pow((double)opt->beta2, (double)(tick ? 1 : opt->t));
        const uint32_t* t_copy = tick ? (const uint32_t*)(slabs + n_slabs * (4 * (int64_t)J + 1)) : nullptr;
        int64_t nb_blk = ((opt->nB + 3) / 4 + 1023) / 1024;
        if (nb_blk > (int64_t)num_cu() * 2) nb_blk = (int64_t)num_cu() * 2;
        if (n_slabs > 512) {
            const int n_red = grid_1d(len, 8);
            hipLaunchKernelGGL(k_reduce_adam<8>, dim3((unsigned)(n_red + nb_blk)), dim3(1024), 0, (hipStream_t)hs, slabs, n_slabs,
                               4 * (int64_t)J + 1, len, -1.0f, gitem, loss, tick, t_copy, (uint32_t)opt->t, A, sa, B, sb, opt->beta1,
                               opt->beta2, opt->eps, (float)bc1, (float)sqrt(bc2), opt->loss_ring, n_red);
        } else {
            const int n_red = grid_1d(len, 32);
            hipLaunchKernelGGL(k_reduce_adam<32>, dim3((unsigned)(n_red + nb_blk)), dim3(1024), 0, (hipStream_t)hs, slabs, n_slabs,
                               4 * (int64_t)J + 1, len, -1.0f, gitem, loss, tick, t_copy, (uint32_t)opt->t, A, sa, B, sb, opt->beta1,
                               opt->beta2, opt->eps, (float)bc1, (float)sqrt(bc2), opt->loss_ring, n_red);
        }
        VX_CHECK_LAUNCH();
        return VX_OK;
    }
    if (n_slabs > 512)
        hipLaunchKernelGGL(k_reduce_wide<8>, dim3(grid_1d(len, 8)), dim3(1024), 0, (hipStream_t)hs, slabs, n_slabs,
                           4 * (int64_t)J + 1, len, -1.0f, gitem, loss, tick);
    else
        hipLaunchKernelGGL(k_reduce_wide<32>, dim3(grid_1d(len, 32)), dim3(1024), 0, (hipStream_t)hs, slabs, n_slabs,
                           4 * (int64_t)J + 1, len, -1.0f, gitem, loss, tick);
    VX_CHECK_LAUNCH();
    return VX_OK;
}

int64_t vx_sum_workspace_floats(void) { return 1024; }

int vx_sum(const float* v, int64_t n, float alpha, float* out, float* workspace, uint32_t* step_dev, void* hs) {
    if (!v || !out || !workspace || n < 0) return VX_EINVAL;
    int nblk = (int)((n + 4095) / 4096);
    if (nblk < 1) nblk = 1;
    if (nblk > 1024) nblk = 1024;
    if (nblk == 1) {
        hipLaunchKernelGGL(k_sum_stage1, dim3(1), dim3(256), 0, (hipStream_t)hs, v, n, workspace, (const float*)nullptr, alpha, out,
                           step_dev);
        VX_CHECK_LAUNCH();
        return VX_OK;
    }
    hipLaunchKernelGGL(k_sum_stage1, dim3(nblk), dim3(256), 0, (hipStream_t)hs, v, n, workspace, (const float*)nullptr);
    VX_CHECK_LAUNCH();
    hipLaunchKernelGGL(k_sum_stage2, dim3(1), dim3(256), 0, (hipStream_t)hs, workspace, nblk, alpha, out, step_dev);
    VX_CHECK_LAUNCH();
    return VX_OK;
}

int vx_sum2(const float* v1, const float* v2, int64_t n, float alpha, float* out, float* workspace, uint32_t* step_dev, void* hs) {
    if (!v1 || !v2 || !out || !workspace || n < 0) return VX_EINVAL;
    int nblk = (int)((n + 4095) / 4096);
    if (nblk < 1) nblk = 1;
    if (nblk > 1024) nblk = 1024;
    if (nblk == 1) {
        hipLaunchKernelGGL(k_sum_stage1, dim3(1), dim3(256), 0, (hipStream_t)hs, v1, n, workspace, v2, alpha, out, step_dev);
        VX_CHECK_LAUNCH();
        return VX_OK;
    }
    hipLaunchKernelGGL(k_sum_stage1, dim3(nblk), dim3(256), 0, (hipStream_t)hs, v1, n, workspace, v2);
    VX_CHECK_LAUNCH();
    hipLaunchKernelGGL(k_sum_stage2, dim3(1), dim3(256), 0, (hipStream_t)hs, workspace, nblk, alpha, out, step_dev);
    VX_CHECK_LAUNCH();
    return VX_OK;
}

int vx_adam_step(float* p, const float* g, float* m, float* v, const float* free_mask, int64_t n,
                 const vx_adam_seg* segs, int32_t n_segs, int32_t t, const uint32_t* t_dev, float beta1, float beta2,
                 float eps, const float* loss_src, float* loss_ring, void* hs) {
    if (!p || !g || !m || !v || !segs || n_segs < 1 || n_segs > VX_MAX_SEGS || (t < 1 && !t_dev) || (loss_ring && !loss_src))
        return VX_EINVAL;
    AdamSegs s;
    s.n = n_segs;
    for (int i = 0; i < n_segs; ++i) {
        if (segs[i].begin < 0 || segs[i].end > n || segs[i].begin > segs[i].end) return VX_EINVAL;
        s.begin[i] = segs[i].begin; s.end[i] = segs[i].end; s.lr[i] = segs[i].lr;
    }
    const double bc1 = 1.0 - pow((double)beta1, (double)(t_dev ? 1 : t));
    const double bc2 = 1.0 - pow((double)beta2, (double)(t_dev ? 1 : t));
    hipLaunchKernelGGL(k_adam, dim3(grid_1d((n + 3) / 4, 256)), dim3(256), 0, (hipStream_t)hs, p, g, m, v, free_mask, n, s,
                       beta1, beta2, eps, (float)bc1, (float)sqrt(bc2), t_dev, (uint32_t)t, loss_src, loss_ring);
    VX_CHECK_LAUNCH();
    return VX_OK;
}

int vx_adam_step2(float* pA, const float* gA, float* mA, float* vA, const float* freeA, int64_t nA, const vx_adam_seg* segsA,
                  int32_t n_segsA, float* pB, const float* gB, float* mB, float* vB, int64_t nB, const vx_adam_seg* segsB,
                  int32_t n_segsB, int32_t t, const uint32_t* t_dev, float beta1, float beta2, float eps, const float* loss_src,
                  float* loss_ring, void* hs) {
    if (!pA || !gA || !mA || !vA || !segsA || !pB || !gB || !mB || !vB || !segsB || n_segsA < 1 || n_segsA > VX_MAX_SEGS ||
        n_segsB < 1 || n_segsB > VX_MAX_SEGS || nA < 0 || nB < 0 || (t < 1 && !t_dev) || (loss_ring && !loss_src))
        return VX_EINVAL;
    AdamSegs sa, sb;
    sa.n = n_segsA; sb.n = n_segsB;
    for (int i = 0; i < n_segsA; ++i) {
        if (segsA[i].begin < 0 || segsA[i].end > nA || segsA[i].begin > segsA[i].end) return VX_EINVAL;
        sa.begin[i] = segsA[i].begin; sa.end[i] = segsA[i].end; sa.lr[i] = segsA[i].lr;
    }
    for (int i = 0; i < n_segsB; ++i) {
        if (segsB[i].begin < 0 || segsB[i].end > nB || segsB[i].begin > segsB[i].end) return VX_EINVAL;
        sb.begin[i] = segsB[i].begin; sb.end[i] = segsB[i].end; sb.lr[i] = segsB[i].lr;
    }
    const AdamBuf A{pA, gA, mA, vA, freeA, nA}, B{pB, gB, mB, vB, nullptr, nB};
    const double bc1 = 1.0 - pow((double)beta1, (double)(t_dev ? 1 : t));
    const double bc2 = 1.0 - pow((double)beta2, (double)(t_dev ? 1 : t));
    hipLaunchKernelGGL(k_adam2, dim3(grid_1d((nA + 3) / 4 + (nB + 3) / 4, 256)), dim3(256), 0, (hipStream_t)hs, A, sa, B, sb, beta1, beta2, eps,
                       (float)bc1, (float)sqrt(bc2), t_dev, (uint32_t)t, loss_src, loss_ring);
    VX_CHECK_LAUNCH();
    return VX_OK;
}

static bool lik_h_shape(const vx_irt_cfg* cfg) {
    return !force_generic() && cfg->D >= 96 && cfg->D <= 16 * LB_NKS - 1 && cfg->model <= VX_IRT_2PL;
}
static int64_t lik_ximg_ovf_bytes(int64_t nb) { return (nb + LB_P - 1) / LB_P * (int64_t)LH_XT_BYTES; }

static int spread(int64_t n_ptiles, int64_t groups) {
    int64_t w = num_cu() / groups;
    if (w < 1) w = 1;
    return (int)(n_ptiles < 1 ? 1 : (n_ptiles < w ? n_ptiles : w));
}

struct PackLayout { int64_t Rp, bp, gtab, wpT, img, gt2, w1img, himg, sc, hscale, maxw, total; };
static PackLayout pack_layout(const vx_irt_cfg* cfg) {
    static_assert(FB_IMG_BYTES % 4 == 0, "the tile images fill whole floats");
    PackLayout l;
    l.Rp = pk_rows(cfg->D);
    l.bp = l.Rp * 64;
    l.gtab = l.bp + l.Rp;
    l.wpT = l.gtab + l.Rp / 8 + 8;
    l.img = l.wpT + l.Rp * 64;
    l.gt2 = l.img + (int64_t)fb_tiles(cfg->D) * (FB_IMG_BYTES / 4);
    l.w1img = l.img + fb_img_floats(cfg->D);
    l.himg = l.w1img + fb_w1img_floats(cfg->J);
    l.sc = l.himg + hb_img_floats(cfg->D);
    l.hscale = l.sc + 3;
    l.maxw = l.sc + 11;
    l.total = l.sc + FB_NSCALES;
    return l;
}

struct MvnPlan {
    bool packed;
    bool fwb;
    bool encb_fast;
    bool bwt;
    bool bwh_t;
    bool bwb;
    bool bwhb;
    bool hb_fw;
    bool fc1_16, side_streams;
    int n_rowslabs, n_prw;
    int n_rowslabs_t, n_prw_t;
    int n_jg, n_prf;
    int n_prw_ws;
    int64_t lenw_ref, lenw, lenf;
    int64_t slabs_w, slabs_f, gd = -1, hs = -1, himg = -1, maxw, total;
};
static MvnPlan mvn_plan(const vx_irt_cfg* cfg, int64_t nb) {
    const Seams& sm = seams();
    const int64_t D = cfg->D, J = cfg->J, H = cfg->H, T = tril_len(cfg->D), Rp = pk_rows(cfg->D);
    MvnPlan p;
    p.packed = packed_ok(cfg);
    p.fwb = fwb_shape(cfg);
    p.encb_fast = !sm.generic && H == 64 && D % 4 == 0 && enc_bwdw_fast_lds_floats(cfg->D) * sizeof(float) <= 160 * 1024;
    p.bwt = p.packed && nb % 4 == 0 && D <= 124 && bt_lds_bytes(cfg->D) <= 160 * 1024;
    p.bwh_t = p.bwt && nb >= 4 && bh_lds_bytes(cfg->D) <= 160 * 1024;
    p.bwb = sm.w16 && p.bwt && nb % 8 == 0 && nb < ((int64_t)1 << 23) && bb_lds_bytes(cfg->D) <= 160 * 1024;
    p.bwhb = sm.h16 && p.bwt && nb >= 4 && D <= 16 * HB_NS && hb_lds_bytes(cfg->D) <= 160 * 1024;
    p.hb_fw = p.fwb && p.bwhb;
    p.fc1_16 = sm.fc1_16;
    p.side_streams = sm.side_streams;
    const int rows_per_wg = p.encb_fast ? BWF_ROWS : BW_ROWS;
    p.n_rowslabs = (int)(((p.packed ? Rp : T + D) + rows_per_wg - 1) / rows_per_wg);
    p.n_jg = (int)((J + FC1_JG - 1) / FC1_JG);
    const int64_t n_ptiles = (nb + ENC_P - 1) / ENC_P;
    p.n_prw = spread(n_ptiles, p.n_rowslabs);
    p.n_prf = spread(n_ptiles, p.n_jg);
    p.n_rowslabs_t = (int)((Rp + BT_ROWS - 1) / BT_ROWS);
    p.n_prw_t = spread((nb + BT_P - 1) / BT_P, p.n_rowslabs_t);
    p.n_prw_ws = (p.bwt && p.n_prw_t > p.n_prw) ? p.n_prw_t : p.n_prw;
    p.lenw_ref = D * H + D + T * H + T;
    p.lenw = (p.packed && Rp * (H + 1) > p.lenw_ref) ? Rp * (H + 1) : p.lenw_ref;
    p.lenf = H * J + H;
    p.slabs_w = nb * H;
    p.slabs_f = p.slabs_w + p.n_prw_ws * p.lenw;
    int64_t end = p.slabs_f + p.n_prf * p.lenf;
    if (p.bwt) { p.gd = end; end += nb * D + 4; }
    if (p.bwb) { p.hs = end; end += nb * 64; }
    if (p.bwhb) { p.himg = end; end += hb_img_floats(cfg->D); }
    p.maxw = end;
    p.total = end + 8;
    return p;
}

static int f1fast_ok(const vx_irt_cfg* cfg, const float* ghpre, const uint8_t* y) {
    return (!force_generic() && cfg->H == 64 && cfg->J % 4 == 0 && aligned16(ghpre) && aligned16(y)) ? 1 : 0;
}

static int mvn_enc_forward_kernels(const vx_irt_cfg* cfg, const MvnPlan& p, bool packed, const uint8_t* y, const int64_t* rows,
                                   int64_t nb, int64_t gid0, const float* W1, const float* b1, const float* W21, const float* b21,
                                   const float* W22, const float* b22, const float* eps_in, float* h, float* x, float* eps,
                                   float* ldT, float* ent, float* hT, float* epsT, float* packws, uint8_t* ximg, uint16_t* hs_out,
                                   void* hs, const int64_t* ring) {
    EncDims dm = make_enc_dims(cfg, nb);
    const dim3 grid((unsigned)((nb + ENC_P - 1) / ENC_P));
    int rc;
    if (packed) {
        const PackLayout pk = pack_layout(cfg);
        float* Wp = packws;
        float* bp = packws + pk.bp;
        uint32_t* gtab = (uint32_t*)(packws + pk.gtab);
        float* WpT = packws + pk.wpT;
        float* sc = packws + pk.sc;
        if (!p.fwb) {
            hipLaunchKernelGGL(k_pack_heads, dim3((unsigned)pk.Rp), dim3(64), 0, (hipStream_t)hs, (int)cfg->D, 64, W21, b21, W22, b22,
                               Wp, bp, gtab, WpT);
            VX_CHECK_LAUNCH();
            hipLaunchKernelGGL(k_clear_words, dim3(1), dim3(64), 0, (hipStream_t)hs, (uint32_t*)(packws + pk.maxw), 4);
            hipLaunchKernelGGL(k_enc_scales_max, dim3(FB_SC_BLOCKS), dim3(256), 0, (hipStream_t)hs, (int)dm.D, (int)dm.J, W1, b1, W21,
                               b21, W22, b22, sc);
            hipLaunchKernelGGL(k_enc_scales, dim3(1), dim3(64), 0, (hipStream_t)hs, sc);
            VX_CHECK_LAUNCH();
        }
        if (p.fwb) {
            uint8_t* img = (uint8_t*)(packws + pk.img);
            const int n_tiles = fb_tiles(dm.D);
            uint32_t* gt2 = (uint32_t*)(packws + pk.gt2);
            uint8_t* w1img = (uint8_t*)(packws + pk.w1img);
            const bool hb = p.hb_fw;
            uint8_t* himg = hb ? (uint8_t*)(packws + pk.himg) : nullptr;
            const bool direct = hb;
            const int n_row_blocks = direct ? 0 : (int)((pk.Rp + 3) / 4), n_w1 = (dm.J + 15) / 16;
            hipLaunchKernelGGL(k_pack_stage1, dim3(n_row_blocks + FB_SC_BLOCKS + (ring ? 1 : 0)), dim3(256), 0, (hipStream_t)hs,
                               (int)dm.D, (int)dm.J, W1, b1, W21, b21, W22, b22, Wp, bp, gtab, hb ? (float*)nullptr : WpT, sc, ring,
                               (int64_t)cfg->rows_ring_stride, (int)cfg->rows_ring_slots, cfg->step_dev, const_cast<int64_t*>(rows),
                               nb, n_row_blocks);
            VX_CHECK_LAUNCH();
            hipLaunchKernelGGL(k_pack_stage2, dim3(n_w1 + n_tiles + (hb ? hb_units(dm.D) : 0)), dim3(256), 0, (hipStream_t)hs,
                               (int)dm.D, (int)dm.J, n_tiles, pk_off_total(dm.D) / 8, W1, W21, W22, (const float*)Wp, (const float*)bp,
                               (const uint32_t*)gtab, sc, w1img, img, gt2, himg, direct ? b21 : (const float*)nullptr,
                               direct ? b22 : (const float*)nullptr, direct ? gtab : (uint32_t*)nullptr);
            VX_CHECK_LAUNCH();
            const size_t ldsb = fb_lds_bytes(dm.D, dm.J);
            if (nb <= FB_SPLIT_MAX) {
                ProfScope ps("k_mvn_enc_fwd_b", (hipStream_t)hs);
                rc = set_lds(k_mvn_enc_fwd_b<true>, ldsb);
                if (rc) return rc;
                const unsigned gs = ximg ? (unsigned)(((nb + 63) / 64) * 2) : (unsigned)((nb + FB_WP - 1) / FB_WP);
                hipLaunchKernelGGL(k_mvn_enc_fwd_b<true>, dim3(gs), dim3(FB_THREADS), ldsb,
                                   (hipStream_t)hs, dm, y, rows, gid0, (const uint8_t*)w1img, b1, (const uint8_t*)img,
                                   (const uint32_t*)gt2, (const float*)sc, eps_in, cfg->seed, cfg->step, cfg->step_dev, cfg->stream, h, x, eps, ldT, ent, hT, epsT, ximg, hs_out);
                VX_CHECK_LAUNCH();
                return VX_OK;
            }
            int64_t n_done = 0;
            constexpr int FNS = 1;
            if (fb2_lds_bytes(dm.D, dm.J, FNS) <= 80 * 1024) {
                const int64_t round2 = (int64_t)FB2_WAVES * 64 * num_cu();
                const int64_t rem = nb % round2;
                n_done = (rem > 0 && 2 * rem <= round2) ? nb - rem : nb;
                n_done -= n_done % (FB2_WAVES * 64);
            }
            ForkScope tail_fork;
            auto launch_tail = [&](hipStream_t ts) -> int {
                int r = set_lds(k_mvn_enc_fwd_b<false>, ldsb);
                if (r) return r;
                ProfScope ps("k_mvn_enc_fwd_b", ts, nb - n_done, ts == (hipStream_t)hs);
                const dim3 gridb((unsigned)((nb - n_done + FB_WAVES * FB_WP - 1) / (FB_WAVES * FB_WP)));
                hipLaunchKernelGGL(k_mvn_enc_fwd_b<false>, gridb, dim3(FB_THREADS), ldsb, ts, dm, y, rows, gid0,
                                   (const uint8_t*)w1img, b1, (const uint8_t*)img, (const uint32_t*)gt2, (const float*)sc, eps_in, cfg->seed,
                                   cfg->step, cfg->step_dev, cfg->stream, h, x, eps, ldT, ent, hT, epsT, ximg, hs_out, n_done);
                VX_CHECK_LAUNCH();
                return VX_OK;
            };
            if (n_done > 0 && n_done < nb && p.side_streams && tail_fork.fork(side_stream(0, (hipStream_t)hs), (hipStream_t)hs)) {
                rc = launch_tail(tail_fork.side());
                if (rc) return rc;
            }
            if (n_done > 0) {
                const bool tile_ring = seams().fwd_ring && fb2s_shape_ok((int)dm.D, (int)dm.J);
                const size_t lds2 = tile_ring ? fb2s_lds_bytes((int)dm.D) : fb2_lds_bytes(dm.D, dm.J, FNS);
                rc = tile_ring ? set_lds(k_mvn_enc_fwd_b2<FNS, true>, lds2) : set_lds(k_mvn_enc_fwd_b2<FNS, false>, lds2);
                if (rc) return rc;
                ProfScope ps("k_mvn_enc_fwd_b2", (hipStream_t)hs, n_done);
                const int wg = FB2_WAVES * 32 * FNS;
                const dim3 grid2((unsigned)((n_done + wg - 1) / wg));
#define LAUNCH_FWD_B2(SH)                                                                                                          \
    hipLaunchKernelGGL((k_mvn_enc_fwd_b2<FNS, SH>), grid2, dim3(FB2_THREADS), lds2, (hipStream_t)hs, dm, y, rows, gid0,          \
                       (const uint8_t*)w1img, b1, (const uint8_t*)img, (const uint32_t*)gt2, (const float*)sc, eps_in, cfg->seed, \
                       cfg->step, cfg->step_dev, cfg->stream, h, x, eps, ldT, ent, hT, epsT, ximg, hs_out)
                if (tile_ring) { LAUNCH_FWD_B2(true); } else { LAUNCH_FWD_B2(false); }
#undef LAUNCH_FWD_B2
                VX_CHECK_LAUNCH();
                if (n_done == nb) return VX_OK;
            }
            if (tail_fork.active()) return tail_fork.join();
            return launch_tail((hipStream_t)hs);
        }
        const size_t ldsp = enc_p_lds_floats(dm.D, dm.J) * sizeof(float);
        rc = set_lds(k_mvn_enc_fwd_p, ldsp);
        if (rc) return rc;
        const dim3 gridp((unsigned)((nb + EP_WAVES * EP_WP - 1) / (EP_WAVES * EP_WP)));
        ProfScope ps("k_mvn_enc_fwd_p", (hipStream_t)hs);
        hipLaunchKernelGGL(k_mvn_enc_fwd_p, gridp, dim3(EP_THREADS), ldsp, (hipStream_t)hs, dm, y, rows, gid0, W1, b1, Wp,
                           bp, gtab, eps_in, cfg->seed, cfg->step, cfg->step_dev, cfg->stream, h, x, eps, ldT, ent, hT, epsT);
        VX_CHECK_LAUNCH();
        return VX_OK;
    }
    if (!force_generic() && cfg->H == 64 && cfg->J % 4 == 0 && aligned16(y) && aligned16(W1) && aligned16(b1) &&
        aligned16(W21) && aligned16(W22) && aligned16(h)) {
        const size_t ldsr = enc_r_lds_floats(dm.D, dm.J) * sizeof(float);
        if (ldsr <= 160 * 1024) {
            rc = set_lds(k_mvn_enc_fwd_r, ldsr);
            if (rc) return rc;
            const dim3 gridr((unsigned)((nb + ER_WAVES * ER_WP - 1) / (ER_WAVES * ER_WP)));
            hipLaunchKernelGGL(k_mvn_enc_fwd_r, gridr, dim3(ER_THREADS), ldsr, (hipStream_t)hs, dm, y, rows, gid0, W1, b1,
                               W21, b21, W22, b22, eps_in, cfg->seed, cfg->step, cfg->step_dev, cfg->stream, h, x, eps, ldT, ent);
            VX_CHECK_LAUNCH();
            return VX_OK;
        }
    }
    const size_t lds = enc_fwd_lds_floats(dm.D, dm.Hp) * sizeof(float);
#define LAUNCH_FWD(HT)                                                                                       \
    rc = set_lds(k_mvn_enc_fwd<HT>, lds);                                                                    \
    if (rc) return rc;                                                                                       \
    hipLaunchKernelGGL(k_mvn_enc_fwd<HT>, grid, dim3(ENC_THREADS), lds, (hipStream_t)hs, dm, y, rows, gid0, W1, \
                       b1, W21, b21, W22, b22, eps_in, cfg->seed, cfg->step, cfg->step_dev, cfg->stream, h, x, eps, ldT, ent)
    if (dm.Hp == 32) { LAUNCH_FWD(1); } else if (dm.Hp == 64) { LAUNCH_FWD(2); } else if (dm.Hp == 96) { LAUNCH_FWD(3); } else { LAUNCH_FWD(4); }
#undef LAUNCH_FWD
    VX_CHECK_LAUNCH();
    return VX_OK;
}

int vx_mvn_enc_forward(const vx_irt_cfg* cfg, const uint8_t* y, const int64_t* rows, int64_t nb, int64_t gid0,
                       const float* W1, const float* b1, const float* W21, const float* b21, const float* W22,
                       const float* b22, const float* eps_in, float* h, float* x, float* eps, float* ldT,
                       float* ent, float* hT, float* epsT, float* packws, uint8_t* ximg, uint16_t* hs_out, void* hs) {
    if (!enc_cfg_ok(cfg) || !y || !W1 || !b1 || !W21 || !b21 || !W22 || !b22 || !h || !x || !eps || !ldT || !ent ||
        nb < 0)
        return VX_EINVAL;
    if (nb == 0) return VX_OK;
    if (ximg && !(lik_h_shape(cfg) && aligned16(ximg))) return VX_EINVAL;
    if (hs_out && (!hT || cfg->H != 64)) return VX_EINVAL;
    const MvnPlan p = mvn_plan(cfg, nb);
    const bool packed = p.packed && packws && aligned16(packws) && aligned16(y) && aligned16(W1) && aligned16(b1) &&
                        aligned16(W21) && aligned16(W22) && aligned16(h);
    if (hs_out && !packed) return VX_EINVAL;
    const bool fused = packed && p.fwb;
    uint32_t* ovf = ximg ? (uint32_t*)(ximg + lik_ximg_ovf_bytes(nb)) : nullptr;
    if (ovf && hipMemsetAsync(ovf, 0, sizeof(uint32_t), (hipStream_t)hs) != hipSuccess) return VX_EINVAL;
    const int64_t* ring = nullptr;
    if (cfg->rows_ring) {
        if (!rows || !cfg->step_dev || cfg->rows_ring_slots < 1 || cfg->rows_ring_stride < nb) return VX_EINVAL;
        void* dp = nullptr;
        if (hipHostGetDevicePointer(&dp, const_cast<int64_t*>(cfg->rows_ring), 0) != hipSuccess || !dp) return VX_EINVAL;
        ring = (const int64_t*)dp;
        if (!fused) {
            hipLaunchKernelGGL(k_rows_from_ring, dim3(1), dim3(256), 0, (hipStream_t)hs, ring, (int64_t)cfg->rows_ring_stride,
                               (int)cfg->rows_ring_slots, cfg->step_dev, const_cast<int64_t*>(rows), nb);
            VX_CHECK_LAUNCH();
            ring = nullptr;
        }
    }
    const int rc = mvn_enc_forward_kernels(cfg, p, packed, y, rows, nb, gid0, W1, b1, W21, b21, W22, b22, eps_in, h, x, eps, ldT,
                                           ent, hT, epsT, packws, ximg, hs_out, hs, ring);
    if (rc) return rc;
    if (ximg && !fused) {
        hipLaunchKernelGGL(k_lik_ximg_h, dim3((unsigned)((nb + LB_P - 1) / LB_P)), dim3(256), 0, (hipStream_t)hs, (int)cfg->D, nb,
                           (const float*)x, ximg, ovf);
        VX_CHECK_LAUNCH();
    }
    if (hs_out && !fused) {
        hipLaunchKernelGGL(k_split2_f16, dim3(num_cu() * 8), dim3(256), 0, (hipStream_t)hs, (const float*)hT, nb * 64,
                           (const float*)(packws + pack_layout(cfg).hscale), hs_out);
        VX_CHECK_LAUNCH();
    }
    return VX_OK;
}

static int xcd_spread(int64_t n_ptiles, int64_t groups) {
    const int n = spread(n_ptiles, groups);
    return n >= 8 ? n & ~7 : n;
}

struct LikPlan {
    bool h;
    bool b;
    bool r;
    int kt, nch;
    int groups, n_pr;
    int64_t slab_len, gx_part, ll_part, gx_tmp;
    int b_groups = 0, b_n_pr = 0;
    int64_t n_ptiles, nbp;
    int64_t b_ximg = -1, b_gx_part = -1, b_ll_part = -1, b_ovf = -1;
    int64_t total;
    int64_t ximg_bytes;
};
static LikPlan lik_plan(const vx_irt_cfg* cfg, int64_t nb) {
    static_assert(LB_XT_BYTES % 4 == 0, "the x image's tiles fill whole floats");
    LikPlan p;
    p.h = lik_h_shape(cfg);
    p.ximg_bytes = p.h ? lik_ximg_ovf_bytes(nb) + LH_FLAG_BYTES : 0;
    p.b = !force_generic() && cfg->D >= 96 && cfg->D <= 16 * LB_NKS - 1;
    p.r = !force_generic() && cfg->D >= 64 && cfg->D <= 127;
    p.slab_len = (int64_t)cfg->D * cfg->J + 3 * (int64_t)cfg->J;
    const int dk = cfg->D + 1;
    p.kt = dk <= 32 ? 1 : (dk <= 64 ? 2 : 4);
    p.nch = cfg->J <= LIK_JC ? 1 : 2;
    if (p.r) {
        p.groups = (cfg->J + LR_JC - 1) / LR_JC;
        p.n_pr = xcd_spread((nb + LR_P - 1) / LR_P, p.groups);
    } else {
        p.groups = (cfg->J + p.nch * LIK_JC - 1) / (p.nch * LIK_JC);
        p.n_pr = spread((nb + LIK_P - 1) / LIK_P, p.groups);
    }
    p.gx_part = (int64_t)p.n_pr * p.slab_len;
    p.ll_part = p.gx_part + (int64_t)p.groups * nb * cfg->D;
    const int64_t used = p.gx_part + (p.groups > 1 ? (int64_t)p.groups * nb * (cfg->D + 1) : 0);
    p.gx_tmp = p.r ? -1 : ((used + 3) & ~(int64_t)3);
    p.total = p.r ? used : used + nb * cfg->D + 4;
    p.n_ptiles = (nb + LB_P - 1) / LB_P;
    p.nbp = p.n_ptiles * LB_P;
    if (p.b) {
        p.b_groups = (cfg->J + LB_JC - 1) / LB_JC;
        p.b_n_pr = xcd_spread(p.n_ptiles, p.b_groups);
        p.b_ximg = ((int64_t)p.b_n_pr * p.slab_len + 3) & ~(int64_t)3;
        p.b_gx_part = p.b_ximg + p.n_ptiles * (LB_XT_BYTES / 4);
        p.b_ll_part = p.b_gx_part + (int64_t)p.b_groups * LB_DP * p.nbp;
        p.b_ovf = p.b_ll_part + (int64_t)p.b_groups * p.nbp;
        if (p.b_ovf + 16 > p.total) p.total = p.b_ovf + 16;
    }
    return p;
}

static bool lik_cfg_ok(const vx_irt_cfg* cfg) {
    return cfg && cfg->D >= 2 && cfg->D <= 127 && cfg->J >= 1 && cfg->model >= VX_IRT_2PL &&
           cfg->model <= VX_IRT_4PL;
}

int64_t vx_irt_lik_ximg_bytes(const vx_irt_cfg* cfg, int64_t nb) {
    if (!lik_cfg_ok(cfg) || nb < 0) return VX_EINVAL;
    return lik_plan(cfg, nb).ximg_bytes;
}

int64_t vx_irt_lik_workspace_floats(const vx_irt_cfg* cfg, int64_t nb) {
    if (!lik_cfg_ok(cfg) || nb < 0) return VX_EINVAL;
    return lik_plan(cfg, nb).total;
}

static int irt_lik_grad_kernels(const vx_irt_cfg* cfg, const uint8_t* y, const int64_t* rows, int64_t nb, const float* x,
                                const float* a, const float* b, const float* c_un, const float* d_un, float* gx, float* gxT,
                                float* ll, float* gitem, float* workspace, const uint8_t* yT, int64_t yT_stride,
                                const uint8_t* ximg_in, const float* epsT, const float* ldT, float* gdT, uint32_t* opmax, void* hs,
                                bool& gd_done) {
    const LikPlan p = lik_plan(cfg, nb);
    const int64_t n_ptiles = p.n_ptiles, nbp = p.nbp;
    if (p.b && !rows && yT && gxT && yT_stride % 64 == 0 && yT_stride >= nbp && aligned16(yT) && nb > 0 && aligned16(workspace) &&
        aligned16(gxT)) {
        const int groups = p.b_groups, n_pr = p.b_n_pr;
        LikBDims dm;
        dm.D = cfg->D; dm.J = cfg->J; dm.model = cfg->model; dm.groups = groups; dm.n_pr = n_pr; dm.gxt = 1;
        dm.Dc = cfg->Dc; dm.scale = cfg->scale; dm.nb = nb;
        dm.slab_len = p.slab_len;
        float* slabs = workspace;
        uint8_t* ximg_ws = (uint8_t*)(workspace + p.b_ximg);
        float* gx_part = workspace + p.b_gx_part;
        const bool f16 = p.h && nbp < ((int64_t)1 << 27);
        const uint8_t* ximg = (f16 && ximg_in && aligned16(ximg_in)) ? ximg_in : ximg_ws;
        float* ll_part = workspace + p.b_ll_part;
        uint32_t* ovf = (ximg == ximg_ws) ? (uint32_t*)(workspace + p.b_ovf)
                                          : (uint32_t*)(const_cast<uint8_t*>(ximg_in) + lik_ximg_ovf_bytes(nb));
        hipStream_t st = (hipStream_t)hs;
        hipError_t he = hipMemsetAsync(slabs, 0, sizeof(float) * (size_t)n_pr * dm.slab_len, st);
        if (he != hipSuccess) return (int)he;
        if (ximg == ximg_ws) {
            if (f16) {
                if (hipMemsetAsync(ovf, 0, sizeof(uint32_t), st) != hipSuccess) return VX_EINVAL;
                hipLaunchKernelGGL(k_lik_ximg_h, dim3((unsigned)n_ptiles), dim3(256), 0, st, (int)cfg->D, nb, x, ximg_ws, ovf);
            } else {
                hipLaunchKernelGGL(k_lik_ximg, dim3((unsigned)n_ptiles), dim3(256), 0, st, (int)cfg->D, nb, x, ximg_ws, (const uint32_t*)nullptr);
            }
            VX_CHECK_LAUNCH();
        }
        int rc;
        const dim3 grid((unsigned)(groups * n_pr));
        if (f16) {
            rc = set_lds(k_irt_lik_h<0>, LH_LDS_BYTES);
            if (rc) return rc;
            ProfScope ps("k_irt_lik_h", st);
            hipLaunchKernelGGL((k_irt_lik_h<0>), grid, dim3(LH_THREADS), LH_LDS_BYTES, st, dm, yT, yT_stride, ximg, a, b,
                               gx_part, ll_part, slabs, (const uint32_t*)ovf);
            VX_CHECK_LAUNCH();
            rc = set_lds(k_irt_lik_b<0>, LB_LDS_BYTES);
            if (rc) return rc;
            hipLaunchKernelGGL(k_lik_ximg, dim3((unsigned)(n_ptiles < 4 * num_cu() ? n_ptiles : 4 * num_cu())), dim3(256), 0, st, (int)cfg->D,
                               nb, x, ximg_ws, (const uint32_t*)ovf);
            hipLaunchKernelGGL((k_irt_lik_b<0>), grid, dim3(LB_THREADS), LB_LDS_BYTES, st, dm, yT, yT_stride, (const uint8_t*)ximg_ws,
                               a, b, c_un, d_un, gx_part, ll_part, slabs, (long long*)nullptr, (const uint32_t*)ovf);
        } else if (cfg->model >= VX_IRT_3PL) {
            rc = set_lds(k_irt_lik_b<1>, LB_LDS_BYTES);
            if (rc) return rc;
            ProfScope ps("k_irt_lik_b", st);
            hipLaunchKernelGGL((k_irt_lik_b<1>), grid, dim3(LB_THREADS), LB_LDS_BYTES, st, dm, yT, yT_stride, ximg,
                               a, b, c_un, d_un, gx_part, ll_part, slabs, (long long*)nullptr);
        } else {
            rc = set_lds(k_irt_lik_b<0>, LB_LDS_BYTES);
            if (rc) return rc;
            ProfScope ps("k_irt_lik_b", st);
            hipLaunchKernelGGL((k_irt_lik_b<0>), grid, dim3(LB_THREADS), LB_LDS_BYTES, st, dm, yT, yT_stride, ximg,
                               a, b, c_un, d_un, gx_part, ll_part, slabs, (long long*)nullptr);
        }
        VX_CHECK_LAUNCH();
        gd_done = true;
        hipLaunchKernelGGL(k_lik_reduce_parts, dim3((unsigned)n_ptiles), dim3(256), (size_t)64 * (cfg->D | 1) * sizeof(float), st, (const float*)gx_part, (const float*)ll_part,
                           x, groups, (int)cfg->D, nb, nbp, cfg->scale, gxT, ll, epsT, ldT, gdT, opmax);
        VX_CHECK_LAUNCH();
        if (gx) {
            hipLaunchKernelGGL(k_transpose, dim3(num_cu() * 8), dim3(256), 0, st, gxT, gx, (int64_t)cfg->D, nb);
            VX_CHECK_LAUNCH();
        }
        return vx_reduce_slabs(slabs, n_pr, dm.slab_len, -1.0f, gitem, hs);
    }
    const int groups = p.groups, n_pr = p.n_pr;
    if (p.r) {
        LikRDims dm;
        dm.D = cfg->D; dm.J = cfg->J; dm.K8 = (cfg->D + 8) & ~7; dm.model = cfg->model;
        { const int nq = dm.K8 >> 3; dm.XS = 8 * (nq <= 13 ? 13 : 16) + 4; }
        dm.groups = groups; dm.n_pr = n_pr; dm.Dc = cfg->Dc; dm.scale = cfg->scale; dm.nb = nb;
        dm.slab_len = p.slab_len;
        dm.fast = (cfg->D % 4 == 0 && cfg->J % 4 == 0 && cfg->J >= 8 && aligned16(x) && aligned16(y) &&
                   aligned16(gx) && aligned16(workspace)) ? 1 : 0;
        dm.gxt = gxT ? 1 : 0;
        float* slabs = workspace;
        float* gx_sum = gxT ? gxT : gx;
        float* gx_part = groups > 1 ? workspace + p.gx_part : gx_sum;
        float* ll_part = groups > 1 ? workspace + p.ll_part : ll;
        hipStream_t st = (hipStream_t)hs;
        const bool finish1 = nb > 0 && groups > 1 && !(gxT && gx);
        if (!finish1) {
            hipError_t he = hipMemsetAsync(slabs, 0, sizeof(float) * (size_t)n_pr * dm.slab_len, st);
            if (he != hipSuccess) return (int)he;
        }
        if (nb > 0) {
            const size_t lds = likr_lds_bytes(dm.XS);
// ... 1420 lines not shown
```

Measured before the change: 109.0.

## Move head bias out of per-tile MFMA into fp32 aux and lower-triangle bias block

Drops the per-tile bias MFMA, which used a broadcast constant fragment, and stores the section-tile bias as fp32 values that initialise the accumulator directly. The off-diagonal b22 lower-triangle contribution is repacked into the aux region of the early tiles and applied as a separate split-f16 MFMA product against the eps vector, scaled per row, when computing the diagonal blocks. This removes one MFMA and one bias fragment load per tile, plus the extra aux DMA in the ring path. The cost is a new per-row eps max scan and an extra triangular bias GEMM per diagonal block. The scale computation also changes, so the score kernel now recomputes its own clamped scales.

```diff
diff --git a/vipsy_amd/csrc/k_mvn_fwd_b.hip b/vipsy_amd/csrc/k_mvn_fwd_b.hip
--- a/vipsy_amd/csrc/k_mvn_fwd_b.hip
+++ b/vipsy_amd/csrc/k_mvn_fwd_b.hip
@@ -83,12 +83,10 @@
 __device__ __forceinline__ void enc_scales_from_max(float mw, float mb, float m1, float l1, float* __restrict__ sc) {
     const float hbound = 1.001f * (fmaxf(l1, 0.f) + log1pf(expf(-fabsf(l1)))) + 1e-30f;
     const int sw1 = f16_scale_exp(m1), sh = f16_scale_exp(hbound);
-    int sw = f16_scale_exp(mw), sb = f16_scale_exp(mb), eb = sw + sh - sb;
-    if (eb > 15) { sw -= eb - 15; eb = 15; }
-    if (eb < -14) { sb = sw + sh + 14; eb = -14; }
+    const int sw = f16_scale_exp(mw), sb = f16_scale_exp(mb);
     sc[0] = ldexpf(1.f, sw1); sc[1] = ldexpf(1.f, -sw1);
     sc[2] = ldexpf(1.f, sw); sc[3] = ldexpf(1.f, sh); sc[4] = ldexpf(1.f, -(sw + sh));
-    sc[5] = ldexpf(1.f, sb); sc[6] = ldexpf(1.f, eb);
+    sc[5] = ldexpf(1.f, sb); sc[6] = ldexpf(1.f, -sb);
     sc[7] = hbound; sc[8] = mw; sc[9] = mb; sc[10] = m1;
 }
 __global__ void k_enc_scales(float* __restrict__ sc) {
@@ -96,12 +94,25 @@
     enc_scales_from_max(sc[11], sc[12], sc[13], sc[14], sc);
 }
 
+__host__ __device__ inline int fb_bx_nks(int D, int kb) {
+    const int a = 2 * kb + 2, b = (D + 15) / 16;
+    return a < b ? a : b;
+}
+__host__ __device__ inline int fb_bx_ks0(int D, int kb) {
+    int n = 0;
+    for (int q = 0; q < kb; ++q) n += fb_bx_nks(D, q);
+    return n;
+}
+__host__ __device__ inline int fb_bx_frags(int D) { return 2 * fb_bx_ks0(D, (D + 31) / 32); }
+__host__ __device__ inline bool fb_bx_ok(int D) { return fb_bx_frags(D) <= pk_off_total(D) / 32; }
+
 template <bool DIRECT = false>
 __device__ __forceinline__ void pack_heads_b_tile(int T, int n_off_groups, const float* __restrict__ Wp, const float* __restrict__ bp,
-                                                  const uint32_t* __restrict__ gtab, float w_scale, float b_scale,
-                                                  uint8_t* __restrict__ img, uint32_t* __restrict__ gt2, int D = 0,
+                                                  const uint32_t* __restrict__ gtab, float w_scale, float b_scale, float h_scale,
+                                                  uint8_t* __restrict__ img, uint32_t* __restrict__ gt2, int D,
+                                                  const float* __restrict__ b22,
                                                   const float* __restrict__ W21 = nullptr, const float* __restrict__ b21 = nullptr,
-                                                  const float* __restrict__ W22 = nullptr, const float* __restrict__ b22 = nullptr,
+                                                  const float* __restrict__ W22 = nullptr,
                                                   uint32_t* __restrict__ gtab_out = nullptr) {
     uint8_t* out = img + (int64_t)T * FB_IMG_BYTES;
     const int tid = threadIdx.x;
@@ -144,13 +155,28 @@
         const int half = lane >> 5;
         v[i] = wrow ? wrow[16 * sx + 8 * (j >> 2) + 4 * half + (j & 3)] : 0.f;
     }
+    const bool sec_tile = 4 * T >= n_off_groups;
     float bv = 0.f;
-    const bool bias_thread = tid < 256 && (tid & 7) < 2;
-    if (bias_thread) {
+    if (sec_tile && (tid & 7) == 0) {
         if constexpr (DIRECT) {
             bv = bsrc < 0 ? 0.f : (bsrc < Tt ? b22[bsrc] : b21[bsrc - Tt]);
         } else {
-            bv = bp[T * 32 + (tid >> 3)];
+            bv = bp[T * 32 + row];
+        }
+    }
+    float tv[2] = {0.f, 0.f};
+    const bool tri_tile = !sec_tile && T < fb_bx_frags(D);
+    if (tri_tile) {
+        int kb = 0;
+        const int ksg = T >> 1;
+        while (ksg >= fb_bx_ks0(D, kb + 1)) ++kb;
+        const int ks = ksg - fb_bx_ks0(D, kb);
+#pragma unroll
+        for (int i = 0; i < 2; ++i) {
+            const int e = tid + 256 * i;
+            const int j = e & 7, lane = e >> 3;
+            const int k = 32 * kb + (lane & 31), l = 16 * ks + 8 * (lane >> 5) + j;
+            if (k < D && l < k) tv[i] = b22[k * (k + 1) / 2 + l];
         }
     }
 #pragma unroll
@@ -160,22 +186,28 @@
         uint16_t* o = (uint16_t*)(out + sx * 1024 + lane * 16) + j;
         split2h_bits(w_scale * v[i], o[0], o[2048]);
     }
-    for (int e = tid; e < FB_AUX_BYTES / 2; e += 256) {
-        const int j = e & 7;
-        uint16_t w = 0;
-        if (e < 256 && j < 2) {
+    uint32_t* aux = (uint32_t*)(out + FB_A_BYTES);
+    if (tri_tile) {
+#pragma unroll
+        for (int i = 0; i < 2; ++i) {
             uint16_t bh, bl;
-            split2h_bits(b_scale * bv, bh, bl);
-            w = j == 0 ? bh : bl;
-        }
-        ((uint16_t*)(out + FB_A_BYTES))[e] = w;
+            split2h_bits(b_scale * tv[i], bh, bl);
+            ((uint16_t*)aux)[tid + 256 * i] = (T & 1) ? bl : bh;
+        }
+    } else {
+        aux[tid] = 0u;
+        if (sec_tile) {
+            __syncthreads();
+            if ((tid & 7) == 0)
+                ((float*)aux)[16 * ((row >> 2) & 1) + (row & 3) + 4 * (row >> 3)] = bv * (w_scale * h_scale);
+        }
     }
 }
 __global__ __launch_bounds__(256) void k_pack_heads_b(int n_tiles, int n_off_groups, const float* __restrict__ Wp, const float* __restrict__ bp,
                                const uint32_t* __restrict__ gtab, const float* __restrict__ sc, uint8_t* __restrict__ img,
-                               uint32_t* __restrict__ gt2) {
+                               uint32_t* __restrict__ gt2, int D, const float* __restrict__ b22) {
     if ((int)blockIdx.x >= n_tiles) return;
-    pack_heads_b_tile(blockIdx.x, n_off_groups, Wp, bp, gtab, sc[2], sc[5], img, gt2);
+    pack_heads_b_tile(blockIdx.x, n_off_groups, Wp, bp, gtab, sc[2], sc[5], sc[3], img, gt2, D, b22);
 }
 
 #define FB_W1_KS 4096
@@ -249,6 +281,52 @@
     fh = __builtin_bit_cast(bf16x8, ph);
     fm = __builtin_bit_cast(bf16x8, pm);
     fl = __builtin_bit_cast(bf16x8, pl);
+}
+
+struct FbBxFrags { f16x8 A[4][2]; };
+__device__ __forceinline__ void fb_bias_load(FbBxFrags& F, const uint8_t* __restrict__ img, int D, int kb, int c, int lane) {
+    const int nks = fb_bx_nks(D, kb);
+    const uint8_t* gb = img + (int64_t)(2 * fb_bx_ks0(D, kb)) * FB_IMG_BYTES + FB_A_BYTES + lane * 16;
+#pragma unroll
+    for (int u = 0; u < 4; ++u) {
+        const int ks = c + u < nks ? c + u : nks - 1;
+#pragma unroll
+        for (int sp = 0; sp < 2; ++sp) F.A[u][sp] = *(const f16x8*)(gb + (int64_t)(2 * ks + sp) * FB_IMG_BYTES);
+    }
+}
+__device__ __forceinline__ f32x16 fb_bias_block(const uint8_t* __restrict__ img, int D, int kb, const float* er, float e_scale,
+                                                int lane, FbBxFrags& F) {
+    const int half = lane >> 5;
+    const int nks = fb_bx_nks(D, kb);
+    f32x16 a = zero16();
+    for (int c = 0; c < nks; c += 4) {
+        if (c > 0) fb_bias_load(F, img, D, kb, c, lane);
+#pragma unroll
+        for (int u = 0; u < 4; ++u) {
+            if (c + u < nks) {
+                float v[8];
+#pragma unroll
+                for (int q = 0; q < 2; ++q) {
+                    const int l0 = 16 * (c + u) + 8 * half + 4 * q;
+                    const f32x4 e = *(const f32x4*)(er + (l0 < D ? l0 : 0));
+#pragma unroll
+                    for (int j = 0; j < 4; ++j) v[4 * q + j] = l0 < D ? e[j] : 0.f;
+                }
+                f16x8 bh, bl;
+                split2h_frag(v, e_scale, bh, bl);
+                a = mfma_f16(F.A[u][1], bh, a);
+                a = mfma_f16(F.A[u][0], bl, a);
+                a = mfma_f16(F.A[u][0], bh, a);
+            }
+        }
+    }
+    return a;
+}
+__device__ __forceinline__ f32x16 fb_bias_block(const uint8_t* __restrict__ img, int D, int kb, const float* er, float e_scale,
+                                                int lane) {
+    FbBxFrags F;
+    fb_bias_load(F, img, D, kb, 0, lane);
+    return fb_bias_block(img, D, kb, er, e_scale, lane, F);
 }
 
 #define FB_SPLIT_MAX 8192
@@ -298,7 +376,7 @@
     uint32_t gtv[FB_GQ];
 #pragma unroll
     for (int q = 0; q < FB_GQ; ++q) { const int e = tid + q * FB_THREADS; gtv[q] = e < 4 * n_off ? gt2[e] : 0u; }
-    const float w1_inv = sc[1], h_scale = sc[3], acc_inv = sc[4];
+    const float w1_inv = sc[1], h_scale = sc[3], acc_inv = sc[4], b_inv = sc[6];
 
     const int n_ydma = (32 * J + 1023) / 1024;
     const bool ydense = !rows && ((J >> 2) & 1) && i0 + FB_WP <= dm.nb && (i0 * J + (int64_t)n_ydma * 1024 <= dm.nb * (int64_t)J) &&
@@ -530,24 +608,27 @@
     float ent_acc = 0.f;
     const float* ep = eps_lds + p * DS;
     float* xp = x_lds + p * DX;
-    struct TileRegs { f16x8 a[2][4]; f16x8 bias; };
+    struct TileRegs { f16x8 a[2][4]; };
     auto pull = [&](TileRegs& R, int t) __attribute__((always_inline)) {
         const int tc = t < t_end ? t : t_end - 1;
         const uint8_t* gb = img + (int64_t)tc * FB_IMG_BYTES + lane * 16;
-        R.bias = *(const f16x8*)(gb + FB_A_BYTES);
 #pragma unroll
         for (int sp = 1; sp >= 0; --sp)
 #pragma unroll
             for (int s = 0; s < 4; ++s) R.a[sp][s] = *(const f16x8*)(gb + (sp * 4 + s) * 1024);
     };
-    f16x8 cfrag;
-    {
-        const _Float16 c16 = (_Float16)sc[6];
-#pragma unroll
-        for (int j = 0; j < 8; ++j) cfrag[j] = c16;
-    }
-    auto mma_all = [&](const TileRegs& R) __attribute__((always_inline)) -> f32x16 {
-        f32x16 a = mfma_f16(R.bias, cfrag, zero16());
+    auto pull_bias = [&](int t) __attribute__((always_inline)) -> f32x16 {
+        const f32x4* bq = (const f32x4*)(img + (int64_t)t * FB_IMG_BYTES + FB_A_BYTES + 64 * half);
+        f32x16 c;
+#pragma unroll
+        for (int g = 0; g < 4; ++g) {
+            const f32x4 q = bq[g];
+#pragma unroll
+            for (int j = 0; j < 4; ++j) c[4 * g + j] = q[j];
+        }
+        return c;
+    };
+    auto mma_all = [&](const TileRegs& R, f32x16 a) __attribute__((always_inline)) -> f32x16 {
 #pragma unroll
         for (int s = 0; s < 4; ++s) a = mfma_f16(R.a[1][s], hb[0][s], a);
 #pragma unroll
@@ -556,6 +637,7 @@
         for (int s = 0; s < 4; ++s) a = mfma_f16(R.a[0][s], hb[0][s], a);
         return a;
     };
+    float e_scale = 1.f, bx_inv = 0.f;
     float cur_part = 0.f;
     const char* ep_h = (const char*)(ep + 4 * half);
     char* xp_b = (char*)xp;
@@ -584,6 +666,16 @@
     FSTAMP();
     __syncthreads();
     FSTAMP();
+    {
+        float m = 0.f;
+        for (int k = 4 * half; k < D; k += 8) {
+            const f32x4 e = *(const f32x4*)(ep + k);
+            m = fmaxf(fmaxf(m, fmaxf(fabsf(e[0]), fabsf(e[1]))), fmaxf(fabsf(e[2]), fabsf(e[3])));
+        }
+        const int se = f16_scale_exp(fmaxf(m, half_swap32(m)));
+        e_scale = ldexpf(1.0f, se);
+        bx_inv = b_inv * ldexpf(1.0f, -se);
+    }
     if constexpr (SPLIT) {
         if (epsT_out && i < dm.nb) {
 #pragma unroll 4
@@ -607,8 +699,7 @@
         EpiOps E;
         if constexpr (!first) epi_read(E, codeP);
         pull(Rn, t + 1);
-        f32x16 a = mfma_f16(Rc.bias, cfrag, zero16());
-        a = mfma_f16(Rc.a[1][0], hb[0][0], a);
+        f32x16 a = mfma_f16(Rc.a[1][0], hb[0][0], zero16());
         a = mfma_f16(Rc.a[1][1], hb[0][1], a);
         if constexpr (!first) epi_group(accP, E.e4[0], codeP.x, 0);
         a = mfma_f16(Rc.a[1][2], hb[0][2], a);
@@ -656,12 +747,16 @@
     auto tile_sec = [&](const f32x16& a, int t2) __attribute__((always_inline)) {
         const bool is_diag = t2 < n_off + n_sec;
         const int k0 = 32 * (t2 - (is_diag ? n_off : n_off + n_sec));
+        f32x16 bx = zero16();
+        if (is_diag && k0 < D) bx = fb_bias_block(img, D, k0 >> 5, ep, e_scale, lane);
 #pragma unroll
         for (int g = 0; g < 4; ++g) {
             const int kk = k0 + 8 * g + 4 * half;
             if (kk < D) {
                 f32x4 xo = *(const f32x4*)(xp + kk);
                 if (is_diag) {
+#pragma unroll
+                    for (int j = 0; j < 4; ++j) xo[j] = fmaf(bx[4 * g + j], bx_inv, xo[j]);
                     const f32x4 ev = *(const f32x4*)(ep + kk);
 #pragma unroll
                     for (int j = 0; j < 4; ++j) {
@@ -681,15 +776,15 @@
     };
     auto sec_iter = [&](TileRegs& Rc, TileRegs& Rn, int t) __attribute__((always_inline)) {
         if (t + 1 < t_end) pull(Rn, t + 1);
-        const f32x16 a = mma_all(Rc);
+        const f32x16 a = mma_all(Rc, pull_bias(t));
         tile_sec(a, t);
     };
     if (SPLIT) {
         for (int ts = wave; ts < n_sec; ts += FB_WAVES) {
             pull(RA, n_off + ts);
-            tile_sec(mma_all(RA), n_off + ts);
+            tile_sec(mma_all(RA, pull_bias(n_off + ts)), n_off + ts);
             pull(RA, n_off + n_sec + ts);
-            tile_sec(mma_all(RA), n_off + n_sec + ts);
+            tile_sec(mma_all(RA, pull_bias(n_off + n_sec + ts)), n_off + n_sec + ts);
         }
         const float ea = ent_acc + __shfl_xor(ent_acc, 32, 64);
         if (half == 0) ent_s[wave * FB_WP + p] = ea;
diff --git a/vipsy_amd/csrc/k_mvn_fwd_b2.hip b/vipsy_amd/csrc/k_mvn_fwd_b2.hip
--- a/vipsy_amd/csrc/k_mvn_fwd_b2.hip
+++ b/vipsy_amd/csrc/k_mvn_fwd_b2.hip
@@ -68,7 +68,7 @@
     const int n_sec = pk_sec(D) / 32;
     const int t_end = n_off + 2 * n_sec;
     for (int e = tid; e < 4 * n_off; e += FB2_THREADS) gt_lds[e] = gt2[e];
-    const float w1_inv = sc[1], h_scale = sc[3], acc_inv = sc[4];
+    const float w1_inv = sc[1], h_scale = sc[3], acc_inv = sc[4], b_inv = sc[6];
     const uint32_t ring_lb = SH ? lds_addr_uniform(ring) : 0u;
     auto ring_dma = [&](int t, int slot) __attribute__((always_inline)) {
         const int tc = t < t_end ? t : t_end - 1;
@@ -76,7 +76,6 @@
         const uint32_t lb = ring_lb + (uint32_t)slot * FB_IMG_BYTES;
         dma16(gb + wave * 1024, lb + (uint32_t)wave * 1024u);
         dma16(gb + (wave + 4) * 1024, lb + (uint32_t)(wave + 4) * 1024u);
-        if (wave == 0) dma16(gb + 8 * 1024, lb + 8u * 1024u);
     };
     if constexpr (SH) { ring_dma(0, 0); ring_dma(1, 1); ring_dma(2, 2); }
 
@@ -303,6 +302,7 @@
         }
     }
     float eps2[NS];
+    float e_scale[NS], bx_inv[NS];
 #pragma unroll
     for (int u = 0; u < NS; ++u) {
         const float* er = eps_lds + (32 * u + p) * DS;
@@ -310,29 +310,36 @@
 #pragma unroll 4
             for (int k = half; k < D; k += 2) epsT_out[(int64_t)k * dm.nb + iu[u]] = er[k];
         }
-        float s2 = 0.f;
-        for (int k = 0; k < D; ++k) s2 = fmaf(er[k], er[k], s2);
+        float s2 = 0.f, em = 0.f;
+        for (int k = 0; k < D; ++k) { s2 = fmaf(er[k], er[k], s2); em = fmaxf(em, fabsf(er[k])); }
         eps2[u] = s2;
+        const int se = f16_scale_exp(em);
+        e_scale[u] = ldexpf(1.0f, se);
+        bx_inv[u] = b_inv * ldexpf(1.0f, -se);
     }
     STAMP();
-    struct TileRegs { f16x8 a[2][4]; f16x8 bias; };
+    struct TileRegs { f16x8 a[2][4]; };
     auto pull = [&](TileRegs& R, int t) __attribute__((always_inline)) {
         const int tc = t < t_end ? t : t_end - 1;
         const uint8_t* gb = img + (int64_t)tc * FB_IMG_BYTES + lane * 16;
-        R.bias = *(const f16x8*)(gb + FB_A_BYTES);
 #pragma unroll
         for (int sp = 1; sp >= 0; --sp)
 #pragma unroll
             for (int s = 0; s < 4; ++s) R.a[sp][s] = *(const f16x8*)(gb + (sp * 4 + s) * 1024);
     };
-    f16x8 cfrag;
-    {
-        const _Float16 c16 = (_Float16)sc[6];
-#pragma unroll
-        for (int j = 0; j < 8; ++j) cfrag[j] = c16;
-    }
-    auto mma_all = [&](const TileRegs& R, int u) __attribute__((always_inline)) -> f32x16 {
-        f32x16 a = mfma_f16(R.bias, cfrag, zero16());
+    auto pull_bias = [&](int t) __attribute__((always_inline)) -> f32x16 {
+        const int tc = t < t_end ? t : t_end - 1;
+        const f32x4* bq = (const f32x4*)(img + (int64_t)tc * FB_IMG_BYTES + FB_A_BYTES + 64 * half);
+        f32x16 c;
+#pragma unroll
+        for (int g = 0; g < 4; ++g) {
+            const f32x4 q = bq[g];
+#pragma unroll
+            for (int j = 0; j < 4; ++j) c[4 * g + j] = q[j];
+        }
+        return c;
+    };
+    auto mma_all = [&](const TileRegs& R, int u, f32x16 a) __attribute__((always_inline)) -> f32x16 {
 #pragma unroll
         for (int s = 0; s < 4; ++s) a = mfma_f16(R.a[1][s], hb[u][0][s], a);
 #pragma unroll
@@ -390,7 +397,6 @@
     int s_rd = 1;
     auto ring_read = [&](TileRegs& R, int slot) __attribute__((always_inline)) {
         const uint8_t* lb = ring + slot * FB_IMG_BYTES + lane * 16;
-        R.bias = *(const f16x8*)(lb + FB_A_BYTES);
 #pragma unroll
         for (int sp = 1; sp >= 0; --sp)
 #pragma unroll
@@ -407,11 +413,9 @@
         if constexpr (SH) ring_read(Rn, s_rd); else pull(Rn, t + 1);
         f32x16 a[NS];
 #pragma unroll
-        for (int u = 0; u < NS; ++u) a[u] = mfma_f16(Rc.bias, cfrag, zero16());
-#pragma unroll
-        for (int s = 0; s < 2; ++s)
-#pragma unroll
-            for (int u = 0; u < NS; ++u) a[u] = mfma_f16(Rc.a[1][s], hb[u][0][s], a[u]);
+        for (int u = 0; u < NS; ++u) a[u] = mfma_f16(Rc.a[1][0], hb[u][0][0], zero16());
+#pragma unroll
+        for (int u = 0; u < NS; ++u) a[u] = mfma_f16(Rc.a[1][1], hb[u][0][1], a[u]);
         if constexpr (!first) epi_group(accP, E, codeP.x, 0);
 #pragma unroll
         for (int s = 2; s < 4; ++s)
@@ -447,7 +451,7 @@
 #ifdef FB2_STAMPS
             const uint64_t tw1_ = __builtin_amdgcn_s_memtime();
 #endif
-            if (wave == 0) __builtin_amdgcn_s_waitcnt(0x0F70 | 3); else __builtin_amdgcn_s_waitcnt(0x0F70 | 2);
+            __builtin_amdgcn_s_waitcnt(0x0F70 | 2);
 #ifdef FB2_STAMPS
             const uint64_t tw2_ = __builtin_amdgcn_s_memtime();
 #endif
@@ -488,9 +492,12 @@
     for (int u = 0; u < NS; ++u) ent_acc[u] = 0.f;
     pull(RA, n_off);
     pull(RB, n_off + n_sec);
+    FbBxFrags BF;
+    fb_bias_load(BF, img, D, 0, 0, lane);
     for (int kb = 0; kb < n_sec; ++kb) {
         const int k0 = 32 * kb;
         if (k0 >= D) break;
+        const f32x16 cD = pull_bias(n_off + kb), cL = pull_bias(n_off + n_sec + kb);
         f32x4 xo[NS][4];
 #pragma unroll
         for (int u = 0; u < NS; ++u) {
@@ -502,12 +509,22 @@
             }
             if (k0 == 0 && half == 0) xo[u][0][0] = 0.f;
         }
+#pragma unroll
+        for (int u = 0; u < NS; ++u) {
+            if (u > 0) fb_bias_load(BF, img, D, kb, 0, lane);
+            const f32x16 bx = fb_bias_block(img, D, kb, eps_lds + (32 * u + p) * DS, e_scale[u], lane, BF);
+#pragma unroll
+            for (int g = 0; g < 4; ++g)
+#pragma unroll
+                for (int j = 0; j < 4; ++j) xo[u][g][j] = fmaf(bx[4 * g + j], bx_inv[u], xo[u][g][j]);
+        }
+        if (32 * (kb + 1) < D) fb_bias_load(BF, img, D, kb + 1, 0, lane);
         f32x16 aD[NS], aL[NS];
 #pragma unroll
-        for (int u = 0; u < NS; ++u) aD[u] = mma_all(RA, u);
+        for (int u = 0; u < NS; ++u) aD[u] = mma_all(RA, u, cD);
         pull(RA, n_off + kb + 1);
 #pragma unroll
-        for (int u = 0; u < NS; ++u) aL[u] = mma_all(RB, u);
+        for (int u = 0; u < NS; ++u) aL[u] = mma_all(RB, u, cL);
         pull(RB, n_off + n_sec + kb + 1);
 #pragma unroll
         for (int u = 0; u < NS; ++u) {
diff --git a/vipsy_amd/csrc/k_mvn_score_b.hip b/vipsy_amd/csrc/k_mvn_score_b.hip
--- a/vipsy_amd/csrc/k_mvn_score_b.hip
+++ b/vipsy_amd/csrc/k_mvn_score_b.hip
@@ -24,12 +24,22 @@
 }
 __host__ __device__ inline int64_t sb_img_floats(int D) { return (int64_t)sb_tiles(D) * (FB_IMG_BYTES / 4); }
 
+struct SbScales { float w_scale, b_scale, acc_inv, cst; };
+__device__ __forceinline__ SbScales sb_scales(const float* __restrict__ sc) {
+    const int sh = f16_scale_exp(sc[7]);
+    int sw = f16_scale_exp(sc[8]), sb = f16_scale_exp(sc[9]), eb = sw + sh - sb;
+    if (eb > 15) { sw -= eb - 15; eb = 15; }
+    if (eb < -14) { sb = sw + sh + 14; eb = -14; }
+    return SbScales{ldexpf(1.f, sw), ldexpf(1.f, sb), ldexpf(1.f, -(sw + sh)), ldexpf(1.f, eb)};
+}
+
 __global__ __launch_bounds__(256) void k_pack_heads_col(int D, const float* __restrict__ W22, const float* __restrict__ b22,
                                                        const float* __restrict__ sc, uint8_t* __restrict__ img) {
     int t = blockIdx.x, c = D - 1;
     while (c > 0 && t >= sb_col_tiles(D, c)) { t -= sb_col_tiles(D, c); --c; }
     const int jb = sb_col_jb0(c) + 32 * t;
-    const float w_scale = sc[2], b_scale = sc[5];
+    const SbScales ss = sb_scales(sc);
+    const float w_scale = ss.w_scale, b_scale = ss.b_scale;
     uint8_t* out = img + (int64_t)blockIdx.x * FB_IMG_BYTES;
     const int tid = threadIdx.x;
     const int row = (tid >> 3) & 31;
@@ -114,7 +124,8 @@
     const int64_t i = i0 + p;
     const bool live = i < nb;
     const int64_t ic = live ? i : nb - 1;
-    const float h_scale = sc[3], acc_inv = sc[4];
+    const SbScales ss = sb_scales(sc);
+    const float h_scale = sc[3], acc_inv = ss.acc_inv;
 
     float w;
     {
@@ -178,7 +189,7 @@
     };
     f16x8 cfrag;
     {
-        const _Float16 c16 = (_Float16)sc[6];
+        const _Float16 c16 = (_Float16)ss.cst;
 #pragma unroll
         for (int j = 0; j < 8; ++j) cfrag[j] = c16;
     }
diff --git a/vipsy_amd/csrc/k_pack_fused.hip b/vipsy_amd/csrc/k_pack_fused.hip
--- a/vipsy_amd/csrc/k_pack_fused.hip
+++ b/vipsy_amd/csrc/k_pack_fused.hip
@@ -59,8 +59,8 @@
                                                      const uint32_t* __restrict__ gtab, float* __restrict__ sc,
                                                      uint8_t* __restrict__ w1img, uint8_t* __restrict__ img, uint32_t* __restrict__ gt2,
                                                      uint8_t* __restrict__ himg ,
-                                                     const float* __restrict__ b21 = nullptr ,
-                                                     const float* __restrict__ b22 = nullptr, uint32_t* __restrict__ gtab_out = nullptr) {
+                                                     const float* __restrict__ b21, const float* __restrict__ b22,
+                                                     uint32_t* __restrict__ gtab_out = nullptr ) {
     __shared__ float scl[16];
     const int tid = threadIdx.x, blk = blockIdx.x;
     if (tid < 64) {
@@ -76,8 +76,8 @@
     const int n_w1 = (J + 15) / 16;
     if (blk < n_w1) { pack_w1_b_kstep(blk, J, W1, scl[0], w1img); return; }
     if (blk < n_w1 + n_tiles) {
-        if (gtab_out) pack_heads_b_tile<true>(blk - n_w1, n_off_groups, Wp, bp, gtab, scl[2], scl[5], img, gt2, D, W21, b21, W22, b22, gtab_out);
-        else pack_heads_b_tile<false>(blk - n_w1, n_off_groups, Wp, bp, gtab, scl[2], scl[5], img, gt2);
+        if (gtab_out) pack_heads_b_tile<true>(blk - n_w1, n_off_groups, Wp, bp, gtab, scl[2], scl[5], scl[3], img, gt2, D, b22, W21, b21, W22, gtab_out);
+        else pack_heads_b_tile<false>(blk - n_w1, n_off_groups, Wp, bp, gtab, scl[2], scl[5], scl[3], img, gt2, D, b22);
         return;
     }
     if (himg) pack_heads_hb_unit(blk - n_w1 - n_tiles, D, W21, W22, scl[2], himg);
diff --git a/vipsy_amd/csrc/vx_abi.hip b/vipsy_amd/csrc/vx_abi.hip
--- a/vipsy_amd/csrc/vx_abi.hip
+++ b/vipsy_amd/csrc/vx_abi.hip
@@ -116,7 +116,7 @@
            enc_bwdw_fast_lds_floats(cfg->D) * sizeof(float) <= 160 * 1024;
 }
 bool fwb_shape(const vx_irt_cfg* cfg) {
-    return seams().fwd16 && packed_ok(cfg) && cfg->D <= 128 && fb_lds_bytes(cfg->D, cfg->J) <= 160 * 1024;
+    return seams().fwd16 && packed_ok(cfg) && cfg->D <= 128 && fb_bx_ok(cfg->D) && fb_lds_bytes(cfg->D, cfg->J) <= 160 * 1024;
 }
 
 bool enc_cfg_ok(const vx_irt_cfg* cfg) {
@@ -565,8 +565,7 @@
             VX_CHECK_LAUNCH();
             hipLaunchKernelGGL(k_pack_stage2, dim3(n_w1 + n_tiles + (hb ? hb_units(dm.D) : 0)), dim3(256), 0, (hipStream_t)hs,
                                (int)dm.D, (int)dm.J, n_tiles, pk_off_total(dm.D) / 8, W1, W21, W22, (const float*)Wp, (const float*)bp,
-                               (const uint32_t*)gtab, sc, w1img, img, gt2, himg, direct ? b21 : (const float*)nullptr,
-                               direct ? b22 : (const float*)nullptr, direct ? gtab : (uint32_t*)nullptr);
+                               (const uint32_t*)gtab, sc, w1img, img, gt2, himg, b21, b22, direct ? gtab : (uint32_t*)nullptr);
             VX_CHECK_LAUNCH();
             const size_t ldsb = fb_lds_bytes(dm.D, dm.J);
             if (nb <= FB_SPLIT_MAX) {
```

New measurement: 109.5, median of 6. Within noise of the previous version (+0.5%).
